# lppllppl920/EndoscopyDepthEstimation-Pytorch

Hardware: AMD Instinct MI355X
Metric: train frame-pairs/sec at 256x320 bs=8 (higher is better)
Workload: dtype f32

## Files before the change

### endoscopydepthestimation-pytorch_amd/csrc/dgrad_newmap_kernels.h

```cpp
#pragma once

#include "dgrad_block_kernels.h"

namespace endo {

template <int NL>
struct NewMapGeom {
    using G = DgradBlockGeom<1, 2, 3, 1, 4>;
    static constexpr int kStage = 12 * G::kCS;
    static constexpr int kW = 9 * 12 * 16;
    static constexpr int kWPre = (kW + kConvThreads - 1) / kConvThreads;
    static constexpr int kConsts = NL * 16 * 4;
    static constexpr size_t kBytes = sizeof(float) * (2 * kStage + NL * kW + kConsts);
    static constexpr int kBlocksPerCu = NL == 1 ? 4 : 3;
    static_assert(kBytes * kBlocksPerCu <= 160 * 1024, "LDS of the resident blocks");
    static_assert(sizeof(double) * 4 * NL * 16 * 2 <= sizeof(float) * kStage, "the final reduction aliases stage 0");
};

template <int NL>
__global__ void __launch_bounds__(kConvThreads, NewMapGeom<NL>::kBlocksPerCu) dgrad_newmap_kernel(const DgradBlockParams p, int tiles_y, int blocks_per_group, int tiles_per_block) {
    using NG = NewMapGeom<NL>;
    using G = typename NG::G;
    constexpr int R = 3;
    extern __shared__ __attribute__((aligned(16))) float smem[];
    float* s_g = smem;
    float* s_w = smem + 2 * NG::kStage;
    float* s_c = s_w + NL * NG::kW;

    const int tid = threadIdx.x;
    const int lane = tid & 63;
    const int wave = __builtin_amdgcn_readfirstlane(tid >> 6);
    const int li = lane & 15;
    const int lk = lane >> 4;
    const int wx = (wave & 1) * 16;
    const int wy = (wave >> 1) * R;

    const int gn = p.group_n > 0 ? p.group_n : p.n;
    const int tps = p.tiles_x * tiles_y;
    const int Q = static_cast<int>(gridDim.x >> 3);
    const bool interleave = (gridDim.x & 7) == 0 && Q > 0 && blocks_per_group % Q == 0;
    int grp, first, t_step, t_last;
    if (interleave) {
        const int lb0 = static_cast<int>(blockIdx.x & 7) * Q;
        grp = lb0 / blocks_per_group;
        const int b0 = lb0 - grp * blocks_per_group;
        first = b0 * tiles_per_block + static_cast<int>(blockIdx.x >> 3);
        t_last = min((b0 + Q) * tiles_per_block, tps * gn);
        t_step = Q;
    } else {
        const int lb = blockIdx.x;
        grp = lb / blocks_per_group;
        first = (lb - grp * blocks_per_group) * tiles_per_block;
        t_last = min(first + tiles_per_block, tps * gn);
        t_step = 1;
    }
    const int ntiles = first < t_last ? (t_last - first + t_step - 1) / t_step : 0;
    if (ntiles <= 0) return;
    const int64_t grp_off = p.group_n > 0 ? grp * p.gs : 0;

    struct Tile { int n, tx, ty, idx; };
    auto place = [&](Tile& t) {
        t.n = t.idx / tps;
        const int rem = t.idx - t.n * tps;
        t.ty = rem / p.tiles_x;
        t.tx = rem - t.ty * p.tiles_x;
    };
    auto advance = [&](Tile& t) { t.idx += t_step; place(t); };
    Tile cur;
    cur.idx = first;
    place(cur);

#pragma unroll
    for (int l = 0; l < NL; ++l) {
        const float* wl = p.wgt[l] + static_cast<int64_t>(p.w_ci_off) * 9;
        const int wcin = p.w_cin[l];
#pragma unroll
        for (int k = 0; k < NG::kWPre; ++k) {
            const int e0 = k * kConvThreads + wave * 64;
            if (e0 < NG::kW) {
                const int e = e0 + lane;
                const int j = e & 15, rest = e >> 4;
                const int tap = rest / 12, cc = rest - tap * 12;
                const bool ok = e < NG::kW && j < p.count;
                const float* src = ok ? wl + cc * 9 * wcin + j * 9 + (8 - tap) : g_pad_consts + 4;
                if (e < NG::kW) __builtin_amdgcn_global_load_lds((gptr_t)src, (lptr_t)(s_w + l * NG::kW + e0), 4, 0, 0);
            }
        }
    }
    const bool co_ok = li < p.count;
    if (tid < NL * 16) {
        const int l = tid >> 4, j = tid & 15;
        const float* sv = p.saved[0];
        const float* ga = p.gamma[0];
        const float* be = p.beta[0];
        if (NL > 1 && l == 1) { sv = p.saved[1]; ga = p.gamma[1]; be = p.beta[1]; }
        if (NL > 2 && l == 2) { sv = p.saved[2]; ga = p.gamma[2]; be = p.beta[2]; }
        f32x4 c4{0.f, 0.f, 0.f, 0.f};
        if (j < p.count) {
            const float mean = sv[grp_off + 2 * j], rstd = sv[grp_off + 2 * j + 1];
            c4 = f32x4{ga[j] * rstd, be[j], mean, rstd};
        }
        *reinterpret_cast<f32x4*>(s_c + tid * 4) = c4;
    }
    const float wfe = p.vg ? (co_ok ? p.vw[li] : 0.f) : 1.f;

    int u_ry[2], u_rx[2];
#pragma unroll
    for (int k = 0; k < 2; ++k) {
        const int u = lane + 64 * k;
        u_ry[k] = u / (G::kCols / 4);
        u_rx[k] = (u - u_ry[k] * (G::kCols / 4)) * 4;
    }
    const bool second_unit = lane + 64 < G::kUnits;
    const unsigned kOob = 0x80000000u;
    unsigned d_vo[2] = {kOob, kOob};
    const float* d_gn = p.g;
    auto dma_tile = [&](const Tile& t) {
        const int x0 = t.tx * G::kTileX, y0 = t.ty * G::kTileY;
#pragma unroll
        for (int k = 0; k < 2; ++k) {
            const int gy = y0 - 1 + u_ry[k], gx = x0 - G::kLeft + u_rx[k];
            const bool ok = gy >= 0 && gy < p.h && gx >= 0 && gx < p.w;
            d_vo[k] = ok ? 4u * static_cast<unsigned>(gy * p.g_w + gx) : kOob;
        }
        d_gn = p.g + grp_off + static_cast<int64_t>(t.n) * p.g_ns;
    };
    auto issue_chunk = [&](int l, int stage) {
        float* dst = s_g + stage * NG::kStage;
        const __amdgpu_buffer_rsrc_t gr = __builtin_amdgcn_make_buffer_rsrc(const_cast<float*>(d_gn), 0, NL * 12 * p.g_cs * 4, 0x00020000);
#pragma unroll
        for (int i = 0; i < 3; ++i) {
            const int c = wave + 4 * i;
            const unsigned so = 4u * static_cast<unsigned>((l * 12 + c) * p.g_cs);
            __builtin_amdgcn_raw_ptr_buffer_load_lds(gr, (lptr_t)(dst + c * G::kCS), 16, d_vo[0], so, 0, 0);
            if (second_unit) __builtin_amdgcn_raw_ptr_buffer_load_lds(gr, (lptr_t)(dst + c * G::kCS + 256), 16, d_vo[1], so, 0, 0);
        }
    };

    f32x4 xc[R], dc[R], total[R];
    const int lane_x = wx + 4 * lk;
    unsigned lo_r[R];
#pragma unroll
    for (int r = 0; r < R; ++r) lo_r[r] = static_cast<unsigned>(li * p.cs + (wy + r) * p.w + lane_x);
    const unsigned lo_ch = static_cast<unsigned>(li * p.cs);
    int64_t cur_off = 0, po_off = 0, cur_voff = 0;
    unsigned cur_rows = 0, po_rows = 0;
    bool cur_full = false, po_full = false;
    auto begin_tile = [&](const Tile& t) {
        const int x0 = t.tx * G::kTileX, y0 = t.ty * G::kTileY;
        cur_full = y0 + G::kTileY <= p.h && x0 + G::kTileX <= p.w;
        cur_off = grp_off + static_cast<int64_t>(t.n) * p.ns + y0 * p.w + x0;
        cur_voff = grp_off + static_cast<int64_t>(t.n) * p.cs + y0 * p.w + x0;
        const float* xb = p.x + cur_off;
        const float* ob = p.vg ? p.vg + cur_voff : p.out + cur_off;
        if (cur_full) {
            cur_rows = co_ok ? 7u : 0u;
#pragma unroll
            for (int r = 0; r < R; ++r) {
                xc[r] = *reinterpret_cast<const f32x4*>(xb + lo_r[r]);
                dc[r] = *reinterpret_cast<const f32x4*>(ob + (p.vg ? lo_r[r] - lo_ch : lo_r[r]));
            }
        } else {
            unsigned rows = 0;
#pragma unroll
            for (int r = 0; r < R; ++r)
                if (y0 + wy + r < p.h) rows |= 1u << r;
            cur_rows = (co_ok && x0 + lane_x + 3 < p.w) ? rows : 0u;
#pragma unroll
            for (int r = 0; r < R; ++r) {
                xc[r] = f32x4{0.f, 0.f, 0.f, 0.f};
                dc[r] = f32x4{0.f, 0.f, 0.f, 0.f};
                if (cur_rows & (1u << r)) {
                    xc[r] = *reinterpret_cast<const f32x4*>(xb + lo_r[r]);
                    dc[r] = *reinterpret_cast<const f32x4*>(ob + (p.vg ? lo_r[r] - lo_ch : lo_r[r]));
                }
            }
        }
    };

    auto store_results = [&]() {
        float* ob = p.out + po_off;
        if (po_full) {
            if (co_ok) {
#pragma unroll
                for (int r = 0; r < R; ++r) *reinterpret_cast<f32x4*>(ob + lo_r[r]) = dc[r];
            }
        } else {
#pragma unroll
            for (int r = 0; r < R; ++r)
                if (po_rows & (1u << r)) *reinterpret_cast<f32x4*>(ob + lo_r[r]) = dc[r];
        }
    };

    constexpr int kFlushTiles = 8;
    float fs1[NL], fs2[NL];
    double ds1[NL], ds2[NL];
    int tiles_since_flush = 0;
#pragma unroll
    for (int l = 0; l < NL; ++l) { fs1[l] = fs2[l] = 0.f; ds1[l] = ds2[l] = 0.0; }
    dma_tile(cur);
    issue_chunk(0, 0);
    Tile nxt = cur;
    advance(nxt);
    int stage = 0;

    for (int t = 0; t < ntiles; ++t) {
#pragma unroll
        for (int l = 0; l < NL; ++l) {
            asm volatile("s_waitcnt vmcnt(0)" ::: "memory");
            __syncthreads();
            if (l == 0) {
                if (t > 0) {
                    store_results();
                }
                begin_tile(cur);
            }
            if (l + 1 < NL) {
                issue_chunk(l + 1, stage ^ 1);
            } else if (t + 1 < ntiles) {
                dma_tile(nxt);
                issue_chunk(0, stage ^ 1);
            }
            f32x4 acc[R];
#pragma unroll
            for (int r = 0; r < R; ++r) acc[r] = f32x4{0.f, 0.f, 0.f, 0.f};
            {
                const float* sg = s_g + stage * NG::kStage;
                const float* wb = s_w + l * NG::kW;
                float av[2][3][R + 2], bw[2][9];
                auto load_quad = [&](int quad, int set) {
                    const float* a_base = sg + (quad * 4 + lk) * G::kCS + wy * G::kCols + wx + li + G::kColOff;
                    const float* b_base = wb + (quad * 4 + lk) * 16 + li;
#pragma unroll
                    for (int r = 0; r < R + 2; ++r)
#pragma unroll
                        for (int dx = 0; dx < 3; ++dx) av[set][dx][r] = a_base[r * G::kCols + dx];
#pragma unroll
                    for (int tap = 0; tap < 9; ++tap) bw[set][tap] = b_base[tap * 12 * 16];
                };
                load_quad(0, 0);
#pragma unroll
                for (int quad = 0; quad < 3; ++quad) {
                    const int set = quad & 1;
                    if (quad + 1 < 3) load_quad(quad + 1, set ^ 1);
                    __builtin_amdgcn_sched_barrier(0);
#pragma unroll
                    for (int dx = 0; dx < 3; ++dx)
#pragma unroll
                        for (int dy = 0; dy < 3; ++dy)
#pragma unroll
                            for (int r = 0; r < R; ++r)
                                acc[r] = __builtin_amdgcn_mfma_f32_16x16x4f32(av[set][dx][r + dy], bw[set][dy * 3 + dx], acc[r], 0, 0, 0);
                    __builtin_amdgcn_sched_barrier(0);
                }
            }
            {
                const f32x4 c4 = *reinterpret_cast<const f32x4*>(s_c + (l * 16 + li) * 4);
                const float scale = c4[0], beta = c4[1], mean = c4[2], rstd = c4[3];
                float s1 = 0.f, s2 = 0.f;
                auto row = [&](int r) {
#pragma unroll
                    for (int e = 0; e < 4; ++e) {
                        const float xcen = xc[r][e] - mean;
                        const float z = fmaf(xcen, scale, beta);
                        const float dz = z > 0.f ? acc[r][e] : 0.f;
                        s1 += dz;
                        s2 = fmaf(dz, xcen, s2);
                        total[r][e] = l == 0 ? scale * dz : fmaf(scale, dz, total[r][e]);
                    }
                };
                if (cur_full) {
#pragma unroll
                    for (int r = 0; r < R; ++r) row(r);
                } else {
#pragma unroll
                    for (int r = 0; r < R; ++r) {
                        if (l == 0) total[r] = f32x4{0.f, 0.f, 0.f, 0.f};
                        if (cur_rows & (1u << r)) row(r);
                    }
                }
                fs1[l] += s1;
                fs2[l] = fmaf(s2, rstd, fs2[l]);
            }
            if (l == NL - 1) {
#pragma unroll
                for (int r = 0; r < R; ++r)
#pragma unroll
                    for (int e = 0; e < 4; ++e) {
                        float old = dc[r][e] * wfe;
                        asm volatile("" : "+v"(old));
                        dc[r][e] = old + total[r][e];
                    }
                po_off = cur_off;
                po_rows = cur_rows;
                po_full = cur_full;
                cur = nxt;
                advance(nxt);
                if (++tiles_since_flush == kFlushTiles) {
                    tiles_since_flush = 0;
#pragma unroll
                    for (int k = 0; k < NL; ++k) {
                        ds1[k] += static_cast<double>(fs1[k]); ds2[k] += static_cast<double>(fs2[k]);
                        fs1[k] = 0.f; fs2[k] = 0.f;
                    }
                }
            }
            stage ^= 1;
            asm volatile("" : "+s"(stage));
        }
    }
    store_results();

    __syncthreads();
    double* red = reinterpret_cast<double*>(smem);
#pragma unroll
    for (int l = 0; l < NL; ++l) {
        double a = ds1[l] + static_cast<double>(fs1[l]), b = ds2[l] + static_cast<double>(fs2[l]);
        a += __shfl_xor(a, 16, 64); a += __shfl_xor(a, 32, 64);
        b += __shfl_xor(b, 16, 64); b += __shfl_xor(b, 32, 64);
        if (lk == 0) {
            red[((wave * NL + l) * 16 + li) * 2] = a;
            red[((wave * NL + l) * 16 + li) * 2 + 1] = b;
        }
    }
    __syncthreads();
    if (tid < 32 * NL) {
        const int l = tid >> 5, j = (tid >> 1) & 15, which = tid & 1;
        if (j < p.count) {
            double t = 0.0;
#pragma unroll
            for (int wv = 0; wv < 4; ++wv) t += red[((wv * NL + l) * 16 + j) * 2 + which];
            double* sc = p.scratch[0];
            if (NL > 1 && l == 1) sc = p.scratch[1];
            if (NL > 2 && l == 2) sc = p.scratch[2];
            atomicAdd(sc + bn_slot_offset(p.slot_stride) + grp_off / 2 + 2 * j + which, t);
        }
    }
}

inline bool dgrad_newmap_ok(const DgradBlockParams& p) {
    return p.count <= 16 && p.acc_from == 0 && 36ll * p.g_cs * 4 < (1ll << 31) && (16ll * p.cs + static_cast<int64_t>(p.h) * p.w) * 4 < (1ll << 32);
}

template <int NL>
inline int launch_dgrad_newmap(DgradBlockParams p, hipStream_t stream) {
    using NG = NewMapGeom<NL>;
    using G = typename NG::G;
    p.tiles_x = (p.w + G::kTileX - 1) / G::kTileX;
    const int tiles_y = (p.h + G::kTileY - 1) / G::kTileY;
    const int groups = p.group_n > 0 ? p.n / p.group_n : 1;
    const int tiles_per_group = p.tiles_x * tiles_y * (p.group_n > 0 ? p.group_n : p.n);
    const int resident = device_cu_count() * NG::kBlocksPerCu / groups;
    const int tiles_per_block = (tiles_per_group + resident - 1) / resident;
    int blocks_per_group = (tiles_per_group + tiles_per_block - 1) / tiles_per_block;
    blocks_per_group = (blocks_per_group + 7) / 8 * 8;
    return launch_dyn(dgrad_newmap_kernel<NL>, dim3(groups * blocks_per_group), kConvThreads, NG::kBytes, stream, p, tiles_y, blocks_per_group, tiles_per_block);
}

}
```

### endoscopydepthestimation-pytorch_amd/csrc/net.hip

```cpp
#include <new>
#include <vector>

#include "dgrad_kernels.h"
#include "dgrad_block_kernels.h"
#include "dgrad_newmap_kernels.h"
#include "td_dgrad_kernels.h"
#include "td_fwd_kernels.h"
#include "wgrad_taps_kernels.h"
#include "wgrad1x1_kernels.h"
#include "wgrad_nsplit_kernels.h"
#include "wgrad_x3_kernels.h"
#include "wgrad_f34_kernels.h"
#include "wgrad_subpix_kernels.h"
#include "wino_fwd_kernels.h"
#include "wino4_fwd_kernels.h"
#include "dgrad_wino_kernels.h"
#include "dgrad_wino3_kernels.h"


namespace endo {

int run_dgrad_wino3_nl4(const DgradBlockParams& p, const float* const* u, hipStream_t stream);
bool dgrad_wino3p_applies(const DgradBlockParams& p);
int run_dgrad_wino3p_nl4(const DgradBlockParams& p, const float* const* u, int blocks, double* fw_parts, int* blocks_used, hipStream_t stream);

constexpr int kGrowth = 12;
constexpr int kLayers = 4;
constexpr int kFirst = 48;
constexpr int kLevels = 5;
constexpr int kNew = kGrowth * kLayers;
constexpr float kBnEps = 1.0e-5f;
constexpr float kBnMomentum = 0.1f;
constexpr int kSideStreamFromLevel = 0;

struct ConvP { int64_t w, b; int cout, cin, ks; int64_t u; int64_t ud; };
struct BnP { int64_t g, b; int c; int64_t run; int64_t saved; };

struct Table {
    ConvP first, final_;
    ConvP down_conv[kLevels][kLayers], td_conv[kLevels], bott_conv[kLayers], tu_conv[kLevels], up_conv[kLevels][kLayers];
    BnP down_bn[kLevels][kLayers], td_bn[kLevels], bott_bn[kLayers], up_bn[kLevels][kLayers];
    std::vector<int64_t> param_offsets;
    std::vector<BnP*> bn_order;
    int64_t param_floats = 0, bn_floats = 0, bn_width_total = 0;
    WinoWeightTable wino;
    WinoWeightTable wino4;
    int64_t wino4_floats = 0;
    int64_t wino_floats = 0;
    WinoDgradTable wino_dgrad;
    int64_t wino_dgrad_floats = 0;
};

inline int down_in(int level) { return kFirst + kNew * level; }
inline int level_channels(int level) { return level < kLevels ? 144 + down_in(level) : 288 + kNew; }

static const Table& table() {
    static Table* t = [] {
        Table* tb = new Table();
        int64_t off = 0;
        auto conv = [&](ConvP& c, int cout, int cin, int ks) {
            c.cout = cout; c.cin = cin; c.ks = ks; c.u = -1; c.ud = -1;
            c.w = off; tb->param_offsets.push_back(off); off += static_cast<int64_t>(cout) * cin * ks * ks;
            c.b = off; tb->param_offsets.push_back(off); off += cout;
        };
        int64_t run = 0, saved = 0;
        auto bn = [&](BnP& b, int c) {
            b.c = c;
            b.g = off; tb->param_offsets.push_back(off); off += c;
            b.b = off; tb->param_offsets.push_back(off); off += c;
            b.run = run; run += 2 * c;
            b.saved = saved; saved += c;
            tb->bn_order.push_back(&b);
        };
        conv(tb->first, kFirst, 3, 3);
        for (int l = 0; l < kLevels; ++l)
            for (int j = 0; j < kLayers; ++j) { bn(tb->down_bn[l][j], down_in(l) + kGrowth * j); conv(tb->down_conv[l][j], kGrowth, down_in(l) + kGrowth * j, 3); }
        for (int l = 0; l < kLevels; ++l) { bn(tb->td_bn[l], down_in(l) + kNew); conv(tb->td_conv[l], down_in(l) + kNew, down_in(l) + kNew, 1); }
        for (int j = 0; j < kLayers; ++j) { bn(tb->bott_bn[j], 288 + kGrowth * j); conv(tb->bott_conv[j], kGrowth, 288 + kGrowth * j, 3); }
        for (int i = 0; i < kLevels; ++i) conv(tb->tu_conv[i], kNew, kNew, 3);
        for (int i = 0; i < kLevels; ++i) {
            const int l = kLevels - 1 - i;
            for (int j = 0; j < kLayers; ++j) { const int cin = 96 + down_in(l) + kGrowth * j; bn(tb->up_bn[i][j], cin); conv(tb->up_conv[i][j], kGrowth, cin, 3); }
        }
        conv(tb->final_, 1, 192, 1);
        tb->param_floats = off;
        tb->bn_floats = run;
        tb->bn_width_total = saved;
        {
            WinoWeightTable& wt = tb->wino;
            wt.layers = 0; wt.start[0] = 0;
            int64_t uoff = 0;
            auto add = [&](ConvP& c) {
                const int l = wt.layers++;
                c.u = uoff;
                wt.cin[l] = c.cin; wt.cout[l] = c.cout; wt.w_off[l] = c.w; wt.u_off[l] = uoff;
                wt.start[l + 1] = wt.start[l] + c.cin * 16;
                uoff += static_cast<int64_t>(c.cin) * kWinoUStride;
            };
            for (int l = 0; l < kLevels; ++l) for (int j = 0; j < kLayers; ++j) add(tb->down_conv[l][j]);
            for (int j = 0; j < kLayers; ++j) add(tb->bott_conv[j]);
            for (int i = 0; i < kLevels; ++i) for (int j = 0; j < kLayers; ++j) add(tb->up_conv[i][j]);
            tb->wino_floats = uoff;
            tb->wino4 = wt;
            int64_t u4 = 0;
            for (int l = 0; l < wt.layers; ++l) { tb->wino4.u_off[l] = u4; u4 += static_cast<int64_t>(wt.cin[l]) * kW4UStride; }
            tb->wino4_floats = u4;
        }
        {
            WinoDgradTable& wd = tb->wino_dgrad;
            wd.layers = 0; wd.start[0] = 0;
            int64_t uoff = 0;
            auto add = [&](ConvP& c, int base) {
                const int l = wd.layers++;
                c.ud = uoff;
                wd.cin[l] = c.cin; wd.groups[l] = base / 16; wd.w_off[l] = c.w; wd.u_off[l] = uoff;
                wd.start[l + 1] = wd.start[l] + 16 * wd.groups[l] * 12;
                uoff += static_cast<int64_t>(wd.groups[l]) * kWinoDgradSlice;
            };
            for (int l = 0; l < kLevels; ++l) for (int j = 0; j < kLayers; ++j) add(tb->down_conv[l][j], down_in(l));
            for (int j = 0; j < kLayers; ++j) add(tb->bott_conv[j], 288);
            for (int i = 0; i < kLevels; ++i) for (int j = 0; j < kLayers; ++j) add(tb->up_conv[i][j], 96 + down_in(kLevels - 1 - i));
            tb->wino_dgrad_floats = uoff;
        }
        return tb;
    }();
    return *t;
}

}

using namespace endo;

struct endo_net {
    int n, h, w;
    int groups;
    int64_t gs;
    struct Level { int h, w, t; int64_t plane; int64_t act, grad; int64_t sums; int64_t pq; } lv[kLevels + 1];
    int64_t pre_off;
    int64_t saved_off;
    int64_t idx_off[kLevels];
    int64_t sums_off;
    int64_t sums_bytes;
    int64_t tape_floats;
    int64_t partial_off;
    int64_t wino_off;
    int64_t wino4_off;
    int64_t pq_off;
    int64_t pq_floats;
    int64_t scratch_off;
    int64_t scratch_bytes;
    int64_t slot_stride;
    int64_t wg_scratch_off;
    int64_t tuw_scratch_off;
    int64_t wd_off;
    int64_t gplane_off;
    int64_t bias_parts_off;
    int64_t fw_parts_off;
    int64_t bias_parts_floats;
    int64_t gradws_floats;
    hipStream_t wstream;
    hipEvent_t ev_fork, ev_join;
    int opt[ENDO_OPT_COUNT];
};

namespace endo {


constexpr int kBiasPartChannels = 2048;
constexpr int kBiasPartLaunches = 64;
constexpr int kFwPartBlocks = 512;
struct BiasReduceTable {
    int n;
    struct Entry { const float* parts; float* bias; int count; int nparts; } e[kBiasPartLaunches];
};
struct BiasParts {
    BiasReduceTable table;
    int64_t used;
};

struct BnFin4 {
    const double* scratch[4];
    const float* saved[4];
    const float* gamma[4];
    float* ggamma[4];
    float* gbeta[4];
};

__global__ void __launch_bounds__(256) prep_dy_kernel(float* __restrict__ dbuf, const float* __restrict__ x, int64_t ns, int plane,
                                                      const float* __restrict__ pq_p, const float* __restrict__ pq_q,
                                                      float* bias_grad, int group_n, int64_t gs, const BnFin4 fin, int nl,
                                                      double count, int training, int64_t slot_stride,
                                                      const float* __restrict__ vg, const float* __restrict__ vw, float* __restrict__ parts) {
    __shared__ double scratch[4];
    const int c = blockIdx.y;
    const int grp = blockIdx.z / group_n, n = blockIdx.z - grp * group_n;
    float pc = pq_p[grp * gs + c], qc = pq_q[grp * gs + c];
    if (nl > 0) {
        const int64_t go = grp * gs;
        double dp = 0.0, dq = 0.0;
#pragma unroll
        for (int j = 0; j < 4; ++j) {
            if (j >= nl) break;
            const double s1 = bn_slot_sum(fin.scratch[j] + go / 2 + 2 * c, slot_stride);
            const double s2 = bn_slot_sum(fin.scratch[j] + go / 2 + 2 * c + 1, slot_stride);
            if (blockIdx.x == 0 && n == 0 && threadIdx.x == 0) {
                atomicAdd(fin.ggamma[j] + c, static_cast<float>(s2));
                atomicAdd(fin.gbeta[j] + c, static_cast<float>(s1));
            }
            if (training) {
                const double mean = fin.saved[j][go + 2 * c], rstd = fin.saved[j][go + 2 * c + 1];
                const double scale = fin.gamma[j][c] * rstd;
                const double k = scale * rstd * s2 / count;
                dp += static_cast<double>(static_cast<float>(-k));
                dq += static_cast<double>(static_cast<float>(-scale * s1 / count + k * mean));
            }
        }
        pc += static_cast<float>(dp);
        qc += static_cast<float>(dq);
    }
    const int64_t base = grp * gs + n * ns + static_cast<int64_t>(c) * plane;
    const float* vg_n = vg ? vg + grp * gs + static_cast<int64_t>(n) * plane : nullptr;
    const float wf = vg ? vw[c] : 0.f;
    float part = 0.f;
    if ((plane & 3) == 0 && !vg_n) {
        const int stride = gridDim.x * blockDim.x * 4;
        int i = (blockIdx.x * blockDim.x + threadIdx.x) * 4;
        for (; i + stride < plane; i += 2 * stride) {
            f32x4 g0 = *reinterpret_cast<const f32x4*>(dbuf + base + i);
            f32x4 g1 = *reinterpret_cast<const f32x4*>(dbuf + base + i + stride);
            const f32x4 x0 = *reinterpret_cast<const f32x4*>(x + base + i);
            const f32x4 x1 = *reinterpret_cast<const f32x4*>(x + base + i + stride);
#pragma unroll
            for (int e = 0; e < 4; ++e) { g0[e] += fmaf(pc, x0[e], qc); part += g0[e]; }
#pragma unroll
            for (int e = 0; e < 4; ++e) { g1[e] += fmaf(pc, x1[e], qc); part += g1[e]; }
            *reinterpret_cast<f32x4*>(dbuf + base + i) = g0;
            *reinterpret_cast<f32x4*>(dbuf + base + i + stride) = g1;
        }
        for (; i < plane; i += stride) {
            f32x4 g = *reinterpret_cast<const f32x4*>(dbuf + base + i);
            const f32x4 xv = *reinterpret_cast<const f32x4*>(x + base + i);
#pragma unroll
            for (int e = 0; e < 4; ++e) { g[e] += fmaf(pc, xv[e], qc); part += g[e]; }
            *reinterpret_cast<f32x4*>(dbuf + base + i) = g;
        }
    } else if ((plane & 3) == 0) {
        for (int i = (blockIdx.x * blockDim.x + threadIdx.x) * 4; i < plane; i += gridDim.x * blockDim.x * 4) {
            f32x4 g;
            if (vg_n) {
                const f32x4 gv = *reinterpret_cast<const f32x4*>(vg_n + i);
                g = f32x4{gv[0] * wf, gv[1] * wf, gv[2] * wf, gv[3] * wf};
            } else {
                g = *reinterpret_cast<const f32x4*>(dbuf + base + i);
            }
            const f32x4 xv = *reinterpret_cast<const f32x4*>(x + base + i);
#pragma unroll
            for (int e = 0; e < 4; ++e) { g[e] += fmaf(pc, xv[e], qc); part += g[e]; }
            *reinterpret_cast<f32x4*>(dbuf + base + i) = g;
        }
    } else {
        for (int i = blockIdx.x * blockDim.x + threadIdx.x; i < plane; i += gridDim.x * blockDim.x) {
            const float g = (vg_n ? vg_n[i] * wf : dbuf[base + i]) + fmaf(pc, x[base + i], qc);
            dbuf[base + i] = g;
            part += g;
        }
    }
    const int lane = threadIdx.x & 63, wave = threadIdx.x >> 6;
    double v = wave_sum(static_cast<double>(part));
    if (lane == 0) scratch[wave] = v;
    __syncthreads();
    if (threadIdx.x == 0 && bias_grad) {
        const float t = static_cast<float>(scratch[0] + scratch[1] + scratch[2] + scratch[3]);
        if (parts) parts[(static_cast<int64_t>(c) * gridDim.z + blockIdx.z) * gridDim.x + blockIdx.x] = t;
        else atomicAdd(bias_grad + c, t);
    }
}

__global__ void __launch_bounds__(256) bias_reduce_kernel(const BiasReduceTable tb) {
    const BiasReduceTable::Entry& e = tb.e[blockIdx.x];
    const int lane = threadIdx.x & 63, wave = threadIdx.x >> 6;
    for (int c = blockIdx.y * 4 + wave; c < e.count; c += gridDim.y * 4) {
        const float* src = e.parts + static_cast<int64_t>(c) * e.nparts;
        double t = 0.0;
        for (int i = lane; i < e.nparts; i += 64) t += static_cast<double>(src[i]);
        t = wave_sum(t);
        if (lane == 0) e.bias[c] += static_cast<float>(t);
    }
}

__global__ void bn_bwd_finalize_kernel(const double* __restrict__ scratch, const float* __restrict__ saved,
                                       const float* __restrict__ gamma, float* __restrict__ ggamma, float* __restrict__ gbeta,
                                       float* __restrict__ pq_p, float* __restrict__ pq_q, int c_count, double count, int training,
                                       int64_t gs, int64_t slot_stride) {
    scratch += blockIdx.y * (gs / 2); saved += blockIdx.y * gs; pq_p += blockIdx.y * gs; pq_q += blockIdx.y * gs;
    for (int c = blockIdx.x * blockDim.x + threadIdx.x; c < c_count; c += gridDim.x * blockDim.x) {
        const double s1 = bn_slot_sum(scratch + 2 * c, slot_stride), s2 = bn_slot_sum(scratch + 2 * c + 1, slot_stride);
        atomicAdd(ggamma + c, static_cast<float>(s2));
        atomicAdd(gbeta + c, static_cast<float>(s1));
        if (training) {
            const double mean = saved[2 * c], rstd = saved[2 * c + 1];
            const double scale = gamma[c] * rstd;
            const double k = scale * rstd * s2 / count;
            pq_p[c] += static_cast<float>(-k);
            pq_q[c] += static_cast<float>(-scale * s1 / count + k * mean);
        }
    }
}

__global__ void bn_bwd_finalize4_kernel(const BnFin4 a, int nl, float* __restrict__ pq_p, float* __restrict__ pq_q, int c_count, double count,
                                        int training, int64_t gs, int64_t slot_stride) {
    const int64_t go = blockIdx.y * gs;
    pq_p += go; pq_q += go;
    for (int c = blockIdx.x * blockDim.x + threadIdx.x; c < c_count; c += gridDim.x * blockDim.x) {
        double dp = 0.0, dq = 0.0;
#pragma unroll
        for (int j = 0; j < 4; ++j) {
            if (j >= nl) break;
            const double s1 = bn_slot_sum(a.scratch[j] + go / 2 + 2 * c, slot_stride);
            const double s2 = bn_slot_sum(a.scratch[j] + go / 2 + 2 * c + 1, slot_stride);
            atomicAdd(a.ggamma[j] + c, static_cast<float>(s2));
            atomicAdd(a.gbeta[j] + c, static_cast<float>(s1));
            if (training) {
                const double mean = a.saved[j][go + 2 * c], rstd = a.saved[j][go + 2 * c + 1];
                const double scale = a.gamma[j][c] * rstd;
                const double k = scale * rstd * s2 / count;
                dp += static_cast<double>(static_cast<float>(-k));
                dq += static_cast<double>(static_cast<float>(-scale * s1 / count + k * mean));
            }
        }
        if (training) {
            pq_p[c] += static_cast<float>(dp);
            pq_q[c] += static_cast<float>(dq);
        }
    }
}

__global__ void tu_phase_weights_kernel(const float* __restrict__ w, int cout, int cin, float* __restrict__ out) {
    constexpr int kPhW = 2 * 12 * 16 + 16;
    const int total = 2 * cin * 2 * 12 * 16;
    for (int i = blockIdx.x * blockDim.x + threadIdx.x; i < total; i += gridDim.x * blockDim.x) {
        const int lane16 = i & 15;
        const int slot = (i >> 4) % 12;
        const int t = (i / (16 * 12)) & 1;
        const int ci = (i / (16 * 12 * 2)) % cin;
        const int a = i / (16 * 12 * 2 * cin);
        int ctap, tile;
        if (slot < 3) { ctap = 0; tile = slot; } else if (slot < 9) { ctap = 1; tile = slot - 3; } else { ctap = 2; tile = slot - 9 + 3; }
        const int b = tile / 3, co = (tile % 3) * 16 + lane16;
        float v = 0.f;
        if (co < cout) {
            const float* src = w + (static_cast<int64_t>(co) * cin + ci) * 9;
            const int ky0 = a == 0 ? (t == 0 ? 0 : 1) : (t == 0 ? 0 : 2), ky1 = a == 0 ? (t == 0 ? 0 : 2) : (t == 0 ? 1 : 2);
            int kx0, kx1;
            if (b == 0) { kx0 = ctap == 0 ? 0 : 1; kx1 = ctap == 0 ? 0 : 2; }
            else { kx0 = ctap == 1 ? 0 : 2; kx1 = ctap == 1 ? 1 : 2; }
            for (int ky = ky0; ky <= ky1; ++ky)
                for (int kx = kx0; kx <= kx1; ++kx) v += src[ky * 3 + kx];
        }
        out[(static_cast<int64_t>(a) * cin + ci) * kPhW + (t * 12 + slot) * 16 + lane16] = v;
    }
}

__global__ void tu_subpix_dgrad_weights_kernel(const float* __restrict__ w, int cout, int cin, float* __restrict__ out) {
    const int pitch = 4 * cin + 16;
    const int total = 4 * cout * 4 * cin;
    for (int i = blockIdx.x * blockDim.x + threadIdx.x; i < total; i += gridDim.x * blockDim.x) {
        const int ci = i % cin;
        const int tap = (i / cin) & 3;
        const int co = (i / (4 * cin)) % cout;
        const int ph = i / (4 * cin * cout);
        const int alpha = ph >> 1, beta = ph & 1, tyi = tap >> 1, txi = tap & 1;
        const int ky0 = alpha == 0 ? (tyi == 0 ? 1 : 0) : (tyi == 0 ? 2 : 0), ky1 = alpha == 0 ? (tyi == 0 ? 2 : 0) : (tyi == 0 ? 2 : 1);
        const int kx0 = beta == 0 ? (txi == 0 ? 1 : 0) : (txi == 0 ? 2 : 0), kx1 = beta == 0 ? (txi == 0 ? 2 : 0) : (txi == 0 ? 2 : 1);
        const float* src = w + (static_cast<int64_t>(co) * cin + ci) * 9;
        float v = 0.f;
        for (int ky = ky0; ky <= ky1; ++ky)
            for (int kx = kx0; kx <= kx1; ++kx) v += src[ky * 3 + kx];
        out[static_cast<int64_t>(ph * cout + co) * pitch + tap * cin + ci] = v;
    }
}

__global__ void __launch_bounds__(256) finalize_partial_kernel(const float* __restrict__ partial, int64_t split_stride, int ksplit,
                                                               int64_t pns, int plane, const float* __restrict__ bias,
                                                               float* __restrict__ out, int64_t out_ns, double* out_sums,
                                                               int group_n, int64_t gs) {
    __shared__ double scratch[2 * 4];
    const int c = blockIdx.y;
    const int grp = blockIdx.z / group_n, n = blockIdx.z - grp * group_n;
    partial += grp * gs; out += grp * gs;
    if (out_sums) out_sums += grp * (gs / 2);
    const float b = bias[c];
    float part[2] = {0.f, 0.f};
    for (int i = blockIdx.x * blockDim.x + threadIdx.x; i < plane; i += gridDim.x * blockDim.x) {
        float v = b;
        for (int s = 0; s < ksplit; ++s) v += partial[s * split_stride + n * pns + static_cast<int64_t>(c) * plane + i];
        out[n * out_ns + static_cast<int64_t>(c) * plane + i] = v;
        part[0] += v;
        part[1] += v * v;
    }
    if (out_sums) block_sum_atomic<2>(part, out_sums + 2 * c, scratch);
}

__global__ void __launch_bounds__(256) final_fwd_kernel(const float* __restrict__ u, int64_t ns, int plane, int cin,
                                                        const float* __restrict__ wgt, const float* __restrict__ bias,
                                                        float* __restrict__ pre, float* __restrict__ out, int group_n, int64_t gs, int c_first) {
    __shared__ float s_w[192];
    for (int c = threadIdx.x; c < cin; c += blockDim.x) s_w[c] = wgt[c];
    __syncthreads();
    const int grp = blockIdx.y / group_n, n = blockIdx.y - grp * group_n;
    u += grp * gs;
    if (pre) pre += grp * gs;
    out += static_cast<int64_t>(grp) * group_n * plane;
    const bool vec = (plane & 3) == 0;
    if (vec) {
        for (int i = (blockIdx.x * blockDim.x + threadIdx.x) * 4; i < plane; i += gridDim.x * blockDim.x * 4) {
            f32x4 acc = {0.f, 0.f, 0.f, 0.f};
            if (c_first > 0) acc = *reinterpret_cast<const f32x4*>(pre + static_cast<int64_t>(n) * plane + i);
            const float* src = u + n * ns + i;
            for (int c = c_first; c < cin; ++c) {
                const f32x4 v = *reinterpret_cast<const f32x4*>(src + static_cast<int64_t>(c) * plane);
                const float wc = s_w[c];
                acc[0] = fmaf(v[0], wc, acc[0]); acc[1] = fmaf(v[1], wc, acc[1]);
                acc[2] = fmaf(v[2], wc, acc[2]); acc[3] = fmaf(v[3], wc, acc[3]);
            }
            const float b = bias[0];
            f32x4 o;
            for (int e = 0; e < 4; ++e) { acc[e] += b; o[e] = fabsf(acc[e]); }
            if (pre) *reinterpret_cast<f32x4*>(pre + static_cast<int64_t>(n) * plane + i) = acc;
            *reinterpret_cast<f32x4*>(out + static_cast<int64_t>(n) * plane + i) = o;
        }
    } else {
        for (int i = blockIdx.x * blockDim.x + threadIdx.x; i < plane; i += gridDim.x * blockDim.x) {
            float acc = c_first > 0 ? pre[static_cast<int64_t>(n) * plane + i] : 0.f;
            for (int c = c_first; c < cin; ++c) acc = fmaf(u[n * ns + static_cast<int64_t>(c) * plane + i], s_w[c], acc);
            acc += bias[0];
            if (pre) pre[static_cast<int64_t>(n) * plane + i] = acc;
            out[static_cast<int64_t>(n) * plane + i] = fabsf(acc);
        }
    }
}

__device__ __forceinline__ float sign_of(float v) { return v > 0.f ? 1.f : (v < 0.f ? -1.f : 0.f); }

__global__ void __launch_bounds__(256) final_g_kernel(const float* __restrict__ gout, const float* __restrict__ pre, float* __restrict__ g,
                                                      int plane, int group_n, int64_t gs) {
    const int grp = blockIdx.y / group_n, n = blockIdx.y - grp * group_n;
    gout += static_cast<int64_t>(blockIdx.y) * plane; pre += grp * gs + static_cast<int64_t>(n) * plane; g += grp * gs + static_cast<int64_t>(n) * plane;
    for (int i = blockIdx.x * blockDim.x + threadIdx.x; i < plane; i += gridDim.x * blockDim.x) g[i] = gout[i] * sign_of(pre[i]);
}

__global__ void __launch_bounds__(256) final_bwd_data_kernel(const float* __restrict__ gout, const float* __restrict__ pre,
                                                             const float* __restrict__ wgt, float* __restrict__ dbuf,
                                                             int64_t ns, int plane, int cin, int group_n, int64_t gs, int c_first) {
    __shared__ float s_w[192];
    for (int c = threadIdx.x; c < cin; c += blockDim.x) s_w[c] = wgt[c];
    __syncthreads();
    const int grp = blockIdx.y / group_n, n = blockIdx.y - grp * group_n;
    gout += static_cast<int64_t>(grp) * group_n * plane; pre += grp * gs; dbuf += grp * gs;
    for (int i = blockIdx.x * blockDim.x + threadIdx.x; i < plane; i += gridDim.x * blockDim.x) {
        const float g = gout[static_cast<int64_t>(n) * plane + i] * sign_of(pre[static_cast<int64_t>(n) * plane + i]);
        for (int c = c_first; c < cin; ++c) dbuf[n * ns + static_cast<int64_t>(c) * plane + i] = g * s_w[c];
    }
}

__global__ void __launch_bounds__(256) final_bwd_weight_kernel(const float* __restrict__ gout, const float* __restrict__ pre,
                                                               const float* __restrict__ u, int64_t ns, int plane, int cin,
                                                               int group_n, int64_t gs, float* __restrict__ gw, float* __restrict__ gb, int c_first) {
    __shared__ double scratch[4];
    const int c = c_first + blockIdx.x;
    const int grp = blockIdx.z / group_n, n = blockIdx.z - grp * group_n;
    const float* gp = gout + static_cast<int64_t>(blockIdx.z) * plane;
    const float* pp = pre + grp * gs + static_cast<int64_t>(n) * plane;
    const float* up = u + grp * gs + n * ns + static_cast<int64_t>(c < cin ? c : 0) * plane;
    float part = 0.f, part2 = 0.f;
    if ((plane & 3) == 0) {
        const int stride = gridDim.y * blockDim.x * 4;
        for (int i = (blockIdx.y * blockDim.x + threadIdx.x) * 4; i < plane; i += stride) {
            const f32x4 gv = *reinterpret_cast<const f32x4*>(gp + i);
            const f32x4 pv = *reinterpret_cast<const f32x4*>(pp + i);
            f32x4 uv = {1.f, 1.f, 1.f, 1.f};
            if (c < cin) uv = *reinterpret_cast<const f32x4*>(up + i);
            part += gv[0] * sign_of(pv[0]) * uv[0] + gv[1] * sign_of(pv[1]) * uv[1];
            part2 += gv[2] * sign_of(pv[2]) * uv[2] + gv[3] * sign_of(pv[3]) * uv[3];
        }
    } else {
        for (int i = blockIdx.y * blockDim.x + threadIdx.x; i < plane; i += gridDim.y * blockDim.x)
            part += gp[i] * sign_of(pp[i]) * (c < cin ? up[i] : 1.f);
    }
    const int lane = threadIdx.x & 63, wave = threadIdx.x >> 6;
    double v = wave_sum(static_cast<double>(part + part2));
    if (lane == 0) scratch[wave] = v;
    __syncthreads();
    if (threadIdx.x == 0) {
        const float t = static_cast<float>(scratch[0] + scratch[1] + scratch[2] + scratch[3]);
        if (c < cin) atomicAdd(gw + c, t); else atomicAdd(gb, t);
    }
}

__global__ void __launch_bounds__(64) final_w_reduce_kernel(const double* __restrict__ parts, int nblocks, int count, float* __restrict__ gw) {
    const int c = blockIdx.x;
    double t = 0.0;
    for (int b = threadIdx.x; b < nblocks; b += 64) t += parts[static_cast<int64_t>(b) * count + c];
    t = wave_sum(t);
    if (threadIdx.x == 0) atomicAdd(gw + c, static_cast<float>(t));
}

constexpr int kBlocks = 2 * kLevels + 1, kDense = kBlocks * kLayers;

enum class DenseFwd { Wino4, Wino2_32x16, Wino2_32x8, SplitK, Direct32x8, Direct16x8, DirectAuto };
struct FwdPlan {
    struct Dense {
        DenseFwd form;
        int stages;
        int ksplit;
        bool chunk_weights;
    } dense[kDense];
    bool bf16;
    bool wino4_weights;
    bool fuse_final;
    bool td_persistent[kLevels];
    bool tu_subpix[kLevels];
};

enum class NewMap { Bf16, Persistent, Vec16, Dword };
enum class BasePass { Block8, Block8Bf16, Wino3, Wino3Persistent, Wino8 };
enum class DenseWgrad { F34, X3, NSplit, Taps, Direct };
enum class TdDgrad { Persistent, Runs128, Dma, Staged };
enum class TuWgrad { Subpix, Taps, Direct };
enum class TuDgrad { Subpix32x8, Subpix16x8, Subpix16x4, Plain };
enum class FirstWgrad { F34Prep, F34, Taps, Direct };
struct BwdPlan {
    struct Block {
        bool fused;
        NewMap newmap[kLayers];
        BasePass base;
        bool wino3_layout;
    } block[kBlocks];
    DenseWgrad wgrad[kDense];
    bool td_wgrad_dma[kLevels];
    TdDgrad td_dgrad[kLevels];
    TuWgrad tu_wgrad[kLevels];
    TuDgrad tu_dgrad[kLevels];
    int overlap;
    bool bf16_wgrad, bf16_dgrad;
    int f34_blocks;
    bool dgrad_weights;
    bool use_virt;
    bool virt_base;
    bool virt_base_w;
    int materialise;
    int c_first;
    FirstWgrad first;
};

struct Ctx {
    const endo_net* net;
    const float* params;
    float* bn_running;
    float* tape;
    float* grads;
    float* gradws;
    int training;
    hipStream_t stream;
    BiasParts* bias_parts = nullptr;
    const float* x = nullptr;
    const FwdPlan* fwd = nullptr;
    const BwdPlan* bwd = nullptr;

    int nt() const { return net->n * net->groups; }
    int fork_wgrad(Ctx& side, int level) const {
        side = *this;
        if (!net->wstream || !bwd->overlap || level < kSideStreamFromLevel) return 0;
        ENDO_CHECK(hipEventRecord(net->ev_fork, stream));
        ENDO_CHECK(hipStreamWaitEvent(net->wstream, net->ev_fork, 0));
        side.stream = net->wstream;
        return 0;
    }
    float* act(int level) const { return tape + net->lv[level].act; }
    float* gbuf(int level) const { return gradws + net->lv[level].grad; }
    double* sums(int level) const { return reinterpret_cast<double*>(reinterpret_cast<char*>(tape) + net->sums_off) + net->lv[level].sums; }
    double* out_sums(int level, int channel) const { return training ? sums(level) + 2 * channel : nullptr; }
    float* saved(const BnP& b) const { return tape + net->saved_off + 2 * b.saved; }
    double* scratch(const BnP& b) const { return reinterpret_cast<double*>(reinterpret_cast<char*>(gradws) + net->scratch_off) + 2 * b.saved; }
    float* pq_p(int level) const { return gradws + net->pq_off + 2 * net->lv[level].pq; }
    float* pq_q(int level) const { return pq_p(level) + net->lv[level].t; }
    uint8_t* idx(int level) const { return reinterpret_cast<uint8_t*>(tape) + net->idx_off[level]; }
};

static void fill_bn_in(const Ctx& c, ConvParams& p, const BnP& b, int level, int ic0) {
    const auto& lv = c.net->lv[level];
    p.in_sums = c.sums(level) + 2 * ic0;
    p.gamma = c.params + b.g;
    p.beta = c.params + b.b;
    p.running_mean = c.bn_running + b.run;
    p.running_var = c.bn_running + b.run + b.c;
    p.saved = c.tape ? c.saved(b) : nullptr;
    p.count = static_cast<double>(c.net->n) * lv.h * lv.w;
    p.eps = kBnEps;
    p.momentum = kBnMomentum;
    p.training = c.training;
}

static void fill_in(const Ctx& c, ConvParams& p, const float* base, int level, int ic0, int cin) {
    const auto& lv = c.net->lv[level];
    p.in = base + ic0 * lv.plane;
    p.in_ns = lv.t * lv.plane;
    p.in_cs = static_cast<int>(lv.plane);
    p.in_w = lv.w;
    p.cin = cin;
}

static void fill_out(const Ctx& c, ConvParams& p, float* base, int level, int oc0, int cout) {
    const auto& lv = c.net->lv[level];
    p.out = base + oc0 * lv.plane;
    p.out_ns = lv.t * lv.plane;
    p.out_cs = static_cast<int>(lv.plane);
    p.out_w = lv.w;
    p.cout = cout;
}

static void fill_grid(const Ctx& c, ConvParams& p, int level) {
    const auto& lv = c.net->lv[level];
    p.n = c.nt(); p.h = lv.h; p.w = lv.w;
    p.group_n = c.net->n; p.gs = c.net->gs; p.in_gs = c.net->gs; p.out_gs = c.net->gs;
}

static double conv_flops(const endo_net* net, int level, int cin, int cout, int ks) {
    return 2.0 * net->n * net->groups * net->lv[level].plane * cin * cout * ks * ks;
}

static void default_options(int (&opt)[ENDO_OPT_COUNT]) {
    opt[ENDO_OPT_WINO_FWD] = 5;
    opt[ENDO_OPT_WINO_DGRAD] = 3;
    opt[ENDO_OPT_DGRAD_VEC] = 2;
    opt[ENDO_OPT_WINO_MIN_TILES] = 1024;
    opt[ENDO_OPT_MFMA_BF16] = 0;
    opt[ENDO_OPT_WGRAD_OVERLAP] = 1;
    opt[ENDO_OPT_MFMA_X3] = 0;
    opt[ENDO_OPT_WGRAD_F34] = 1;
    opt[ENDO_OPT_FINAL_VIRTUAL] = 1;
    opt[ENDO_OPT_TD_PERSIST] = 3;
}
static int bf16_mask(const int* opt) { const int v = opt[ENDO_OPT_MFMA_BF16]; return v == 1 ? 7 : (v >> 1); }

struct DenseBlock { int level, ic0, c0; const BnP* bn; const ConvP* cv; bool base_overwrite; };
static DenseBlock dense_block(int b) {
    const Table& tb = table();
    if (b < kLevels) return {b, 48, down_in(b), tb.down_bn[b], tb.down_conv[b], false};
    if (b == kLevels) return {kLevels, 0, 288, tb.bott_bn, tb.bott_conv, true};
    const int i = b - kLevels - 1, l = kLevels - 1 - i;
    return {l, 0, 96 + down_in(l), tb.up_bn[i], tb.up_conv[i], l > 0};
}
static long tile_count(const Ctx& c, int level, int tx, int ty) {
    const auto& lv = c.net->lv[level];
    return static_cast<long>((lv.w + tx - 1) / tx) * ((lv.h + ty - 1) / ty) * c.nt();
}

static ConvParams dense_fwd_params(const Ctx& c, const DenseBlock& k, int j, DenseFwd form) {
    const ConvP& cv = k.cv[j];
    const int oc0 = k.ic0 + k.c0 + kGrowth * j;
    ConvParams p{};
    fill_grid(c, p, k.level);
    fill_in(c, p, c.act(k.level), k.level, k.ic0, cv.cin);
    fill_bn_in(c, p, k.bn[j], k.level, k.ic0);
    p.wgt = c.params + cv.w; p.bias = c.params + cv.b; p.w_cout = cv.cout; p.w_cin = cv.cin;
    fill_out(c, p, c.act(k.level), k.level, oc0, cv.cout);
    p.out_sums = c.out_sums(k.level, oc0);
    if (form == DenseFwd::Wino4) p.wgt = c.tape + c.net->wino4_off + cv.u / kWinoUStride * kW4UStride;
    if (form == DenseFwd::Wino2_32x16 || form == DenseFwd::Wino2_32x8) p.wgt = c.tape + c.net->wino_off + cv.u;
    return p;
}

static ConvParams td_fwd_params(const Ctx& c, int level) {
    const BnP& b = table().td_bn[level];
    const ConvP& cv = table().td_conv[level];
    const int next = level + 1;
    const int oc0 = next < kLevels ? 48 : 0;
    ConvParams p{};
    fill_grid(c, p, level);
    fill_in(c, p, c.act(level), level, 48, cv.cin);
    fill_bn_in(c, p, b, level, 48);
    p.wgt = c.params + cv.w; p.bias = c.params + cv.b; p.w_cout = cv.cout; p.w_cin = cv.cin;
    fill_out(c, p, c.act(next), next, oc0, cv.cout);
    p.out_idx = c.idx(level);
    p.idx_ns = static_cast<int64_t>(cv.cout) * c.net->lv[next].plane;
    p.out_sums = c.out_sums(next, oc0);
    return p;
}

static FwdPlan plan_fwd(const Ctx& c) {
    const int* opt = c.net->opt;
    const int mode = opt[ENDO_OPT_WINO_FWD];
    const long min_tiles = opt[ENDO_OPT_WINO_MIN_TILES];
    FwdPlan pl{};
    pl.bf16 = (bf16_mask(opt) & 2) != 0;
    pl.wino4_weights = !pl.bf16 && mode == 5;
    for (int b = 0; b < kBlocks; ++b) {
        const DenseBlock k = dense_block(b);
        const long t64x16 = tile_count(c, k.level, 64, 16), t32x16 = tile_count(c, k.level, 32, 16), t32x8 = tile_count(c, k.level, 32, 8);
        const long t16x16 = tile_count(c, k.level, 16, 16), t16x8 = tile_count(c, k.level, 16, 8);
        const bool big = t32x16 >= min_tiles, small = t32x8 >= (min_tiles * 3) / 4;
        const bool wino4_tiles = mode == 5 && !pl.bf16 && 2 * t64x16 >= min_tiles;
        const bool wino2_tiles = mode != 0 && !pl.bf16 && (big || small);
        for (int j = 0; j < kLayers; ++j) {
            FwdPlan::Dense& d = pl.dense[b * kLayers + j];
            const int nchunks = (k.cv[j].cin + 15) / 16;
            d.chunk_weights = !pl.bf16 && !wino4_tiles && !wino2_tiles;
            d.stages = mode == 4 ? 4 : (mode == 3 ? 3 : 2);
            if (wino4_tiles && wino4_fwd_ok(dense_fwd_params(c, k, j, DenseFwd::Wino4))) {
                d.form = DenseFwd::Wino4;
            } else if (wino2_tiles && wino_fwd_ok(dense_fwd_params(c, k, j, DenseFwd::Wino2_32x16))) {
                d.form = big ? DenseFwd::Wino2_32x16 : DenseFwd::Wino2_32x8;
            } else if (t32x16 < 512 && t16x16 < 384 && t16x8 < 512 && nchunks >= 4) {
                int want = static_cast<int>(((t16x8 < 256 ? 512 : 768) + t16x8 - 1) / t16x8);
                if (want > nchunks) want = nchunks;
                const int per = (nchunks + want - 1) / want;
                d.form = DenseFwd::SplitK;
                d.ksplit = (nchunks + per - 1) / per;
            } else {
                d.form = (t32x16 < 1024 && t32x8 >= 1024) ? DenseFwd::Direct32x8
                       : (t32x16 < 1024 && t16x8 >= 768) ? DenseFwd::Direct16x8 : DenseFwd::DirectAuto;
            }
        }
    }
    pl.fuse_final = opt[ENDO_OPT_FINAL_VIRTUAL] && pl.dense[kDense - 1].form == DenseFwd::Wino4;
    for (int l = 0; l < kLevels; ++l) {
        pl.td_persistent[l] = (opt[ENDO_OPT_TD_PERSIST] & 2) && !pl.bf16 && c.training && td_fwd_ok(td_fwd_params(c, l));
        const ConvP& tu = table().tu_conv[kLevels - 1 - l];
        pl.tu_subpix[l] = c.net->lv[l + 1].w % 4 == 0 && tu.cout == kNew && tu.cin % 4 == 0;
    }
    return pl;
}

static int dense_fwd(const Ctx& c, int b, int j) {
    const DenseBlock k = dense_block(b);
    const FwdPlan::Dense& d = c.fwd->dense[b * kLayers + j];
    const ConvP& cv = k.cv[j];
    const auto& lv = c.net->lv[k.level];
    const int oc0 = k.ic0 + k.c0 + kGrowth * j;
    ConvParams p = dense_fwd_params(c, k, j, d.form);
    ProfScope prof(kProfConv3x3Dense, c.stream, conv_flops(c.net, k.level, cv.cin, cv.cout, 3),
                   4.0 * c.nt() * lv.plane * (cv.cin + cv.cout));
    const float* chunk_weights = d.chunk_weights ? c.tape + c.net->wino_off + cv.u : nullptr;
    const bool bf16 = c.fwd->bf16;
    switch (d.form) {
        case DenseFwd::Wino4:
            if (c.fwd->fuse_final && b == kBlocks - 1 && j == kLayers - 1) { p.fin_w = c.params + table().final_.w + k.ic0; p.fin_out = c.tape + c.net->pre_off; }
            return launch_wino4_fwd(p, c.stream);
        case DenseFwd::Wino2_32x16:
            return d.stages == 4 ? launch_wino_fwd<2, 4, 2, 4>(p, c.stream) : d.stages == 3 ? launch_wino_fwd<2, 4, 2, 3>(p, c.stream) : launch_wino_fwd<2, 4, 2, 2>(p, c.stream);
        case DenseFwd::Wino2_32x8:
            return d.stages == 4 ? launch_wino_fwd<1, 4, 3, 4>(p, c.stream) : d.stages == 3 ? launch_wino_fwd<1, 4, 3, 3>(p, c.stream) : launch_wino_fwd<1, 4, 3, 2>(p, c.stream);
        case DenseFwd::SplitK: {
            float* partial = c.tape + c.net->partial_off;
            p.ksplit = d.ksplit;
            p.split_stride = static_cast<int64_t>(c.net->n) * cv.cout * lv.plane;
            p.out = partial; p.out_ns = static_cast<int64_t>(cv.cout) * lv.plane;
            p.bias = nullptr; p.out_sums = nullptr;
            p.wgt_chunks = chunk_weights;
            int rc = bf16 ? launch_conv_dma<3, 16, 1, IN_BNRELU, EPI_FWD, 1, 2, 2, 1, 1>(p, c.stream)
                          : launch_conv_dma<3, 16, 1, IN_BNRELU, EPI_FWD, 1, 2, 2, 1>(p, c.stream);
            if (rc) return rc;
            int bx = static_cast<int>((lv.plane + 255) / 256);
            bx = bx > 8 ? 8 : bx;
            finalize_partial_kernel<<<dim3(bx, cv.cout, c.nt()), 256, 0, c.stream>>>(
                partial, p.split_stride, d.ksplit, p.out_ns, static_cast<int>(lv.plane), c.params + cv.b, c.act(k.level) + oc0 * lv.plane,
                lv.t * lv.plane, c.out_sums(k.level, oc0), c.net->n, c.net->gs);
            ENDO_LAUNCH_CHECK();
            return 0;
        }
        case DenseFwd::Direct32x8:
            return bf16 ? launch_conv_dma<3, 4, 1, IN_BNRELU, EPI_FWD, 2, 4, 2, 1, 1>(p, c.stream) : launch_conv_dma<3, 4, 1, IN_BNRELU, EPI_FWD, 2, 4, 2, 1>(p, c.stream);
        case DenseFwd::Direct16x8:
            return bf16 ? launch_conv_dma<3, 8, 1, IN_BNRELU, EPI_FWD, 1, 2, 2, 1, 1>(p, c.stream) : launch_conv_dma<3, 8, 1, IN_BNRELU, EPI_FWD, 1, 2, 2, 1>(p, c.stream);
        case DenseFwd::DirectAuto:
            if (bf16) return launch_conv_dma_auto<3, 4, 1, IN_BNRELU, EPI_FWD, 8, 2, 1, 1>(p, c.stream);
            p.wgt_chunks = chunk_weights;
            return launch_conv_dma_auto<3, 4, 1, IN_BNRELU, EPI_FWD, 8, 2, 1>(p, c.stream);
    }
    return ENDO_E_BADARG;
}

static int td_fwd(const Ctx& c, int level) {
    const ConvP& cv = table().td_conv[level];
    const ConvParams p = td_fwd_params(c, level);
    ProfScope prof(kProfConv1x1Pool, c.stream, conv_flops(c.net, level, cv.cin, cv.cout, 1),
                   4.0 * c.nt() * c.net->lv[level].plane * (cv.cin + cv.cout / 4.0));
    if (c.fwd->td_persistent[level]) return launch_td_fwd(p, device_cu_count(), c.stream);
    if (c.fwd->bf16) return launch_conv_dma_auto<1, 8, 3, IN_BNRELU, EPI_FWD_POOL, 4, 2, 1, 1>(p, c.stream);
    return launch_conv_dma_auto<1, 8, 3, IN_BNRELU, EPI_FWD_POOL, 4>(p, c.stream);
}

static int tu_fwd(const Ctx& c, int level, int src_level, int src_c0, const ConvP& cv) {
    ProfScope prof(kProfConv3x3Up, c.stream, conv_flops(c.net, level, cv.cin, cv.cout, 3),
                   4.0 * c.nt() * c.net->lv[level].plane * (cv.cin / 4.0 + cv.cout));
    if (c.fwd->tu_subpix[level]) {
        float* w3 = c.tape + c.net->partial_off;
        tu_phase_weights_kernel<<<(2 * cv.cin * 384 + 255) / 256, 256, 0, c.stream>>>(c.params + cv.w, cv.cout, cv.cin, w3);
        ENDO_LAUNCH_CHECK();
        ConvParams p{};
        fill_grid(c, p, src_level);
        fill_in(c, p, c.act(src_level), src_level, src_c0, cv.cin);
        p.wgt = w3; p.w_cout = 2 * cv.cout; p.w_cin = cv.cin;
        p.bias = c.params + cv.b;
        fill_out(c, p, c.act(level), level, 0, cv.cout);
        p.out_sums = c.out_sums(level, 0);
        return launch_conv_dma_vec<3, 4, 6, IN_PLAIN, EPI_FWD, 2, 4, 2, 1, 4, 0, 0, 2>(p, c.stream);
    }
    ConvParams p{};
    fill_grid(c, p, level);
    fill_in(c, p, c.act(src_level), src_level, src_c0, cv.cin);
    p.wgt = c.params + cv.w; p.bias = c.params + cv.b; p.w_cout = cv.cout; p.w_cin = cv.cin;
    fill_out(c, p, c.act(level), level, 0, cv.cout);
    p.out_sums = c.out_sums(level, 0);
    return launch_conv_dma_auto<3, 4, 3, IN_UPSAMPLE, EPI_FWD>(p, c.stream);
}

struct FinalVirt { const float* vg; const float* vw; float* gw; };

static int prep_dy(const Ctx& c, int level, int c0, int count, float* bias_grad, const BnFin4* fin = nullptr, int nl = 0, const FinalVirt* fv = nullptr) {
    const auto& lv = c.net->lv[level];
    BnFin4 none{};
    int bx = static_cast<int>((lv.plane + 4095) / 4096);
    bx = bx < 1 ? 1 : (bx > 32 ? 32 : bx);
    float* parts = nullptr;
    if (bias_grad && c.bias_parts) {
        BiasParts& bp = *c.bias_parts;
        const int64_t need = static_cast<int64_t>(count) * c.nt() * bx;
        if (bp.table.n >= kBiasPartLaunches || bp.used + need > c.net->bias_parts_floats) return ENDO_E_UNSUPPORTED;
        parts = c.gradws + c.net->bias_parts_off + bp.used;
        bp.table.e[bp.table.n++] = {parts, bias_grad, count, c.nt() * bx};
        bp.used += need;
    }
    ProfScope prof(kProfSmall, c.stream, 0.0, 12.0 * c.nt() * lv.plane * count);
    prep_dy_kernel<<<dim3(bx, count, c.nt()), 256, 0, c.stream>>>(c.gbuf(level) + c0 * lv.plane, c.act(level) + c0 * lv.plane,
                                                                     lv.t * lv.plane, static_cast<int>(lv.plane), c.pq_p(level) + c0,
                                                                     c.pq_q(level) + c0, bias_grad, c.net->n, c.net->gs, fin ? *fin : none, fin ? nl : 0,
                                                                     static_cast<double>(c.net->n) * lv.h * lv.w, c.training, c.net->slot_stride,
                                                                     fv ? fv->vg : nullptr, fv ? fv->vw + c0 : nullptr, parts);
    ENDO_LAUNCH_CHECK();
    return 0;
}

static int bn_finalize(const Ctx& c, const BnP& b, int level, int ic0, int first = 0, int count = -1) {
    const auto& lv = c.net->lv[level];
    if (count < 0) count = b.c - first;
    if (count <= 0) return 0;
    ProfScope prof(kProfSmall, c.stream, 0.0, 0.0);
    bn_bwd_finalize_kernel<<<dim3((count + 127) / 128, c.net->groups), 128, 0, c.stream>>>(c.scratch(b) + 2 * first, c.saved(b) + 2 * first, c.params + b.g + first,
                                                                       c.grads + b.g + first, c.grads + b.b + first,
                                                                       c.pq_p(level) + ic0 + first, c.pq_q(level) + ic0 + first, count,
                                                                       static_cast<double>(c.net->n) * lv.h * lv.w, c.training, c.net->gs, c.net->slot_stride);
    ENDO_LAUNCH_CHECK();
    return 0;
}

static void fill_wgrad_grid(const Ctx& c, WgradParams& p, int level) {
    const auto& lv = c.net->lv[level];
    p.n = c.nt(); p.h = lv.h; p.w = lv.w;
    p.group_n = c.net->n; p.gs = c.net->gs; p.in_gs = c.net->gs;
    p.tiles_x = (lv.w + kWgTileX - 1) / kWgTileX;
    p.tiles_y = (lv.h + kWgTileY - 1) / kWgTileY;
}

static WgradParams dense_wgrad_params(const Ctx& c, const DenseBlock& k, int j) {
    const auto& lv = c.net->lv[k.level];
    const BnP& b = k.bn[j];
    const ConvP& cv = k.cv[j];
    const int oc0 = k.ic0 + k.c0 + kGrowth * j;
    WgradParams p{};
    fill_wgrad_grid(c, p, k.level);
    p.in = c.act(k.level) + k.ic0 * lv.plane; p.in_ns = lv.t * lv.plane; p.in_cs = static_cast<int>(lv.plane); p.in_w = lv.w; p.cin = cv.cin;
    p.saved = c.saved(b); p.gamma = c.params + b.g; p.beta = c.params + b.b;
    p.dy = c.gbuf(k.level) + oc0 * lv.plane; p.dy_ns = lv.t * lv.plane; p.dy_cs = static_cast<int>(lv.plane); p.dy_w = lv.w; p.cout = cv.cout;
    p.dw = c.grads + cv.w;
    return p;
}

static void fill_dgrad_block(const Ctx& c, DgradBlockParams& p, int level) {
    const auto& lv = c.net->lv[level];
    p.n = c.nt(); p.h = lv.h; p.w = lv.w;
    p.group_n = c.net->n; p.gs = c.net->gs; p.slot_stride = c.net->slot_stride;
    p.g_ns = lv.t * lv.plane; p.g_cs = static_cast<int>(lv.plane); p.g_w = lv.w;
    p.ns = lv.t * lv.plane; p.cs = static_cast<int>(lv.plane);
}

static DgradBlockParams newmap_params(const Ctx& c, const DenseBlock& k, int j, BnFin4* a = nullptr) {
    const auto& lv = c.net->lv[k.level];
    const int nl = kLayers - j;
    const int t0 = k.c0 + kGrowth * (j - 1);
    DgradBlockParams p{};
    fill_dgrad_block(c, p, k.level);
    p.g = c.gbuf(k.level) + (k.ic0 + k.c0 + kGrowth * j) * lv.plane;
    p.x = c.act(k.level) + (k.ic0 + t0) * lv.plane;
    p.out = c.gbuf(k.level) + (k.ic0 + t0) * lv.plane;
    p.count = kGrowth;
    p.acc_from = 0;
    p.w_ci_off = t0;
    for (int l = 0; l < nl; ++l) {
        const BnP& b = k.bn[j + l];
        p.wgt[l] = c.params + k.cv[j + l].w; p.w_cin[l] = k.cv[j + l].cin;
        p.saved[l] = c.saved(b) + 2 * t0; p.gamma[l] = c.params + b.g + t0; p.beta[l] = c.params + b.b + t0;
        p.scratch[l] = c.scratch(b) + 2 * t0;
        if (a) { a->scratch[l] = p.scratch[l]; a->saved[l] = p.saved[l]; a->gamma[l] = p.gamma[l]; a->ggamma[l] = c.grads + b.g + t0; a->gbeta[l] = c.grads + b.b + t0; }
    }
    return p;
}

static DgradBlockParams base_pass_params(const Ctx& c, const DenseBlock& k) {
    const auto& lv = c.net->lv[k.level];
    DgradBlockParams p{};
    fill_dgrad_block(c, p, k.level);
    p.g = c.gbuf(k.level) + (k.ic0 + k.c0) * lv.plane;
    p.x = c.act(k.level) + k.ic0 * lv.plane;
    p.out = c.gbuf(k.level) + k.ic0 * lv.plane;
    p.count = k.c0;
    p.acc_from = k.base_overwrite ? k.c0 : 0;
    p.w_ci_off = 0;
    for (int j = 0; j < kLayers; ++j) {
        p.wgt[j] = c.params + k.cv[j].w; p.w_cin[j] = k.cv[j].cin;
        p.saved[j] = c.saved(k.bn[j]); p.gamma[j] = c.params + k.bn[j].g; p.beta[j] = c.params + k.bn[j].b;
        p.scratch[j] = c.scratch(k.bn[j]);
    }
    return p;
}

static WgradParams td_wgrad_params(const Ctx& c, int level) {
    const BnP& b = table().td_bn[level];
    const ConvP& cv = table().td_conv[level];
    const int next = level + 1, oc0 = next < kLevels ? 48 : 0;
    const auto& lv = c.net->lv[level];
    const auto& nx = c.net->lv[next];
    WgradParams p{};
    fill_wgrad_grid(c, p, level);
    p.in = c.act(level) + 48 * lv.plane; p.in_ns = lv.t * lv.plane; p.in_cs = static_cast<int>(lv.plane); p.in_w = lv.w; p.cin = cv.cin;
    p.saved = c.saved(b); p.gamma = c.params + b.g; p.beta = c.params + b.b;
    p.dy = c.gbuf(next) + oc0 * nx.plane; p.dy_ns = nx.t * nx.plane; p.dy_cs = static_cast<int>(nx.plane); p.dy_w = nx.w; p.cout = cv.cout;
    p.dy_idx = c.idx(level); p.idx_ns = static_cast<int64_t>(cv.cout) * nx.plane;
    p.dw = c.grads + cv.w;
    return p;
}

static ConvParams td_dgrad_params(const Ctx& c, int level) {
    const BnP& b = table().td_bn[level];
    const ConvP& cv = table().td_conv[level];
    const int next = level + 1, oc0 = next < kLevels ? 48 : 0;
    const auto& lv = c.net->lv[level];
    ConvParams p{};
    fill_grid(c, p, level);
    fill_in(c, p, c.gbuf(next), next, oc0, cv.cout);
    p.in_idx = c.idx(level); p.idx_ns = static_cast<int64_t>(cv.cout) * c.net->lv[next].plane;
    p.wgt = c.params + cv.w; p.w_cout = cv.cout; p.w_cin = cv.cin;
    fill_out(c, p, c.gbuf(level), level, 48, cv.cin);
    p.x = c.act(level) + 48 * lv.plane; p.x_ns = lv.t * lv.plane; p.x_cs = static_cast<int>(lv.plane);
    p.bn_saved = c.saved(b); p.bn_gamma = c.params + b.g; p.bn_beta = c.params + b.b;
    p.bn_scratch = c.scratch(b); p.bn_slot_stride = c.net->slot_stride;
    p.acc_from = 0;
    return p;
}

static WgradParams tu_wgrad_params(const Ctx& c, int level, bool subpix) {
    const ConvP& cv = table().tu_conv[kLevels - 1 - level];
    const int src_level = level + 1, src_c0 = src_level == kLevels ? 288 : 96 + down_in(src_level);
    const auto& lv = c.net->lv[level];
    const auto& sv = c.net->lv[src_level];
    WgradParams p{};
    fill_wgrad_grid(c, p, level);
    p.in = c.act(src_level) + src_c0 * sv.plane; p.in_ns = sv.t * sv.plane; p.in_cs = static_cast<int>(sv.plane); p.in_w = sv.w; p.cin = cv.cin;
    p.dy = c.gbuf(level); p.dy_ns = lv.t * lv.plane; p.dy_cs = static_cast<int>(lv.plane); p.dy_w = lv.w; p.cout = cv.cout;
    p.dw = c.grads + cv.w;
    if (subpix) { p.h = sv.h; p.w = sv.w; }
    return p;
}

static WgradParams first_wgrad_params(const Ctx& c) {
    const auto& lv = c.net->lv[0];
    WgradParams p{};
    fill_wgrad_grid(c, p, 0);
    p.in = c.x; p.in_ns = 3 * lv.plane; p.in_cs = static_cast<int>(lv.plane); p.in_w = lv.w; p.cin = 3;
    p.in_gs = c.net->n * p.in_ns;
    p.dy = c.gbuf(0) + 48 * lv.plane; p.dy_ns = lv.t * lv.plane; p.dy_cs = static_cast<int>(lv.plane); p.dy_w = lv.w; p.cout = kFirst;
    p.dw = c.grads + table().first.w;
    return p;
}

static BwdPlan plan_bwd(const Ctx& c) {
    const int* opt = c.net->opt;
    const int wino_dgrad = opt[ENDO_OPT_WINO_DGRAD];
    const long min_tiles = opt[ENDO_OPT_WINO_MIN_TILES];
    BwdPlan pl{};
    pl.overlap = opt[ENDO_OPT_WGRAD_OVERLAP];
    pl.bf16_wgrad = (bf16_mask(opt) & 1) != 0;
    pl.bf16_dgrad = (bf16_mask(opt) & 4) != 0;
    const bool x3 = !pl.bf16_wgrad && (opt[ENDO_OPT_MFMA_X3] & 1);
    const bool f34 = opt[ENDO_OPT_WGRAD_F34] && !pl.bf16_wgrad && !x3;
    const long f34_min_tiles = min_tiles / 4;
    pl.f34_blocks = opt[ENDO_OPT_WGRAD_F34] == 2 ? 256 : kF34Blocks;
    pl.dgrad_weights = wino_dgrad != 0 && !pl.bf16_dgrad;
    for (int b = 0; b < kBlocks; ++b) {
        const DenseBlock k = dense_block(b);
        const auto& lv = c.net->lv[k.level];
        BwdPlan::Block& bl = pl.block[b];
        const DgradBlockParams base = base_pass_params(c, k);
        bl.fused = dgrad_block_ok(base);
        const long wtiles = static_cast<long>(lv.w / 32) * (lv.h / 8) * c.nt();
        if (pl.bf16_dgrad) bl.base = BasePass::Block8Bf16;
        else if (wino_dgrad != 0 && dgrad_wino_ok(base) && wtiles >= min_tiles)
            bl.base = !((wino_dgrad == 1 || wino_dgrad == 3) && dgrad_wino3_ok(base)) ? BasePass::Wino8
                    : (wino_dgrad == 3 && dgrad_wino3p_applies(base)) ? BasePass::Wino3Persistent : BasePass::Wino3;
        else bl.base = BasePass::Block8;
        bl.wino3_layout = bl.base == BasePass::Wino3 || bl.base == BasePass::Wino3Persistent;
        for (int j = 1; j < kLayers; ++j) {
            const DgradBlockParams p = newmap_params(c, k, j);
            const bool vec = dgrad_block_vec_ok(p);
            bl.newmap[j] = (pl.bf16_dgrad && vec) ? NewMap::Bf16 : (vec && opt[ENDO_OPT_DGRAD_VEC] >= 2 && dgrad_newmap_ok(p)) ? NewMap::Persistent
                         : (vec && opt[ENDO_OPT_DGRAD_VEC] != 0) ? NewMap::Vec16 : NewMap::Dword;
        }
        for (int j = 0; j < kLayers; ++j) {
            const WgradParams p = dense_wgrad_params(c, k, j);
            pl.wgrad[b * kLayers + j] = (f34 && wgrad_f34_ok(p, f34_min_tiles)) ? DenseWgrad::F34 : wgrad_nsplit_ok(p) ? (x3 ? DenseWgrad::X3 : DenseWgrad::NSplit)
                                      : wgrad_taps_ok(p) ? DenseWgrad::Taps : DenseWgrad::Direct;
        }
    }
    for (int l = 0; l < kLevels; ++l) {
        const auto& sv = c.net->lv[l + 1];
        pl.td_wgrad_dma[l] = wgrad1x1_dma_ok(td_wgrad_params(c, l));
        const ConvParams td = td_dgrad_params(c, l);
        const bool persist = (opt[ENDO_OPT_TD_PERSIST] & 1) && !pl.bf16_dgrad;
        pl.td_dgrad[l] = (persist && td_dgrad_ok(td)) ? TdDgrad::Persistent : (persist && sv.w % 4 != 0 && td_dgrad_small_ok(td)) ? TdDgrad::Runs128
                       : sv.w % 4 == 0 ? TdDgrad::Dma : TdDgrad::Staged;
        const ConvP& tu = table().tu_conv[kLevels - 1 - l];
        pl.tu_wgrad[l] = tu_wgrad_subpix_ok(tu_wgrad_params(c, l, true)) ? TuWgrad::Subpix : wgrad_taps_ok(tu_wgrad_params(c, l, false), true) ? TuWgrad::Taps : TuWgrad::Direct;
        pl.tu_dgrad[l] = !(sv.w % 4 == 0 && tu.cin == kNew && tu.cout == kNew) ? TuDgrad::Plain : tile_count(c, l + 1, 32, 8) >= 1024 ? TuDgrad::Subpix32x8
                       : tile_count(c, l + 1, 16, 8) >= 512 ? TuDgrad::Subpix16x8 : TuDgrad::Subpix16x4;
    }
    const BwdPlan::Block& last = pl.block[kBlocks - 1];
    const int last_base = dense_block(kBlocks - 1).c0;
    pl.use_virt = opt[ENDO_OPT_FINAL_VIRTUAL] && last.fused;
    pl.virt_base = pl.use_virt && last.wino3_layout;
    pl.virt_base_w = pl.use_virt && last.base == BasePass::Wino3Persistent;
    pl.materialise = !pl.use_virt ? 192 : (pl.virt_base ? 0 : last_base);
    pl.c_first = pl.virt_base_w ? last_base : 0;
    const WgradParams first = first_wgrad_params(c);
    pl.first = (f34 && wgrad_f34_raw_ok(first, f34_min_tiles)) ? (opt[ENDO_OPT_FINAL_VIRTUAL] ? FirstWgrad::F34Prep : FirstWgrad::F34)
             : wgrad_taps_ok(first) ? FirstWgrad::Taps : FirstWgrad::Direct;
    return pl;
}

static int dense_wgrad(const Ctx& c, int b, int j, F34ReduceBatch* batch = nullptr, int slice = 0) {
    const DenseBlock k = dense_block(b);
    const ConvP& cv = k.cv[j];
    const auto& lv = c.net->lv[k.level];
    const WgradParams p = dense_wgrad_params(c, k, j);
    float* scratch = c.gradws + c.net->wg_scratch_off;
    ProfScope prof(kProfWgradDense, c.stream, conv_flops(c.net, k.level, cv.cin, cv.cout, 3), 4.0 * c.nt() * lv.plane * (cv.cin + cv.cout));
    switch (c.bwd->wgrad[b * kLayers + j]) {
        case DenseWgrad::F34: return launch_wgrad_f34(p, scratch + (batch ? slice : 0) * kF34ScratchFloats, c.stream, c.bwd->f34_blocks, batch);
        case DenseWgrad::X3: return launch_wgrad_x3(p, scratch, c.stream);
        case DenseWgrad::NSplit: return launch_wgrad_nsplit(p, scratch, c.stream, c.bwd->bf16_wgrad ? 1 : 0);
        case DenseWgrad::Taps: return c.bwd->bf16_wgrad ? launch_wgrad_taps<12, IN_BNRELU, 1>(p, c.stream) : launch_wgrad_taps<12, IN_BNRELU>(p, c.stream);
        case DenseWgrad::Direct: return launch_wgrad<3, 1, IN_BNRELU, DY_PLAIN>(p, c.stream);
    }
    return ENDO_E_BADARG;
}

static int dense_bwd(const Ctx& c, int b, int j, int acc_from) {
    const DenseBlock k = dense_block(b);
    const BnP& bn = k.bn[j];
    const ConvP& cv = k.cv[j];
    const int level = k.level, ic0 = k.ic0, oc0 = k.ic0 + k.c0 + kGrowth * j;
    const auto& lv = c.net->lv[level];
    int rc = prep_dy(c, level, oc0, cv.cout, c.grads + cv.b);
    if (rc) return rc;
    {
        Ctx cw;
        rc = c.fork_wgrad(cw, level);
        if (rc) return rc;
        rc = dense_wgrad(cw, b, j);
        if (rc) return rc;
    }
    {
        ConvParams p{};
        fill_grid(c, p, level);
        fill_in(c, p, c.gbuf(level), level, oc0, cv.cout);
        p.wgt = c.params + cv.w; p.w_cout = cv.cout; p.w_cin = cv.cin;
        fill_out(c, p, c.gbuf(level), level, ic0, cv.cin);
        p.x = c.act(level) + ic0 * lv.plane; p.x_ns = lv.t * lv.plane; p.x_cs = static_cast<int>(lv.plane);
        p.bn_saved = c.saved(bn); p.bn_gamma = c.params + bn.g; p.bn_beta = c.params + bn.b;
        p.bn_scratch = c.scratch(bn); p.bn_slot_stride = c.net->slot_stride;
        p.acc_from = acc_from - ic0;
        ProfScope prof(kProfDgradDense, c.stream, conv_flops(c.net, level, cv.cin, cv.cout, 3), 4.0 * c.nt() * lv.plane * (3.0 * cv.cin + cv.cout));
        rc = launch_dgrad_dense_auto(p, c.stream);
        if (rc) return rc;
    }
    return bn_finalize(c, bn, level, ic0);
}

template <int NL>
static int launch_newmap(NewMap form, const DgradBlockParams& p, hipStream_t stream) {
    switch (form) {
        case NewMap::Bf16: return launch_dgrad_block<NL, 2, 3, 1, 0, 1, 4, 1>(p, stream);
        case NewMap::Persistent: return launch_dgrad_newmap<NL>(p, stream);
        case NewMap::Vec16: return launch_dgrad_block<NL, 2, 3, 1, 0, 1, 4>(p, stream);
        case NewMap::Dword: return launch_dgrad_block<NL, 2, 3>(p, stream);
    }
    return ENDO_E_BADARG;
}

static int dense_block_bwd(const Ctx& c, int b, const FinalVirt* fv = nullptr) {
    const DenseBlock k = dense_block(b);
    const BwdPlan::Block& bl = c.bwd->block[b];
    const int level = k.level, ic0 = k.ic0, c0 = k.c0, new0 = ic0 + c0;
    const auto& lv = c.net->lv[level];
    if (!bl.fused) {
        for (int j = kLayers - 1; j >= 0; --j) {
            const int acc_from = (j == kLayers - 1 && k.base_overwrite) ? new0 : 0;
            int rc = dense_bwd(c, b, j, acc_from < ic0 ? ic0 : acc_from);
            if (rc) return rc;
        }
        return 0;
    }
    BnFin4 pending{};
    int pending_nl = 0;
    F34ReduceBatch red{};
    for (int j = kLayers - 1; j >= 0; --j) {
        int rc = prep_dy(c, level, new0 + kGrowth * j, kGrowth, c.grads + k.cv[j].b, &pending, pending_nl, (fv && j == kLayers - 1) ? fv : nullptr);
        if (rc) return rc;
        const bool defer = c.bwd->overlap == 2;
        if (!defer || j == 0) {
            Ctx cw;
            rc = c.fork_wgrad(cw, level);
            if (rc) return rc;
            for (int jj = defer ? kLayers - 1 : j; jj >= j; --jj) {
                rc = dense_wgrad(cw, b, jj, &red, jj);
                if (rc) return rc;
            }
            if (j == 0 && red.count > 0) {
                ProfScope prof(kProfSmall, cw.stream, 0.0, 0.0);
                rc = launch_wgrad_f34_reduce_batch(red, cw.stream);
                if (rc) return rc;
            }
        }
        if (j > 0) {
            const int nl = kLayers - j;
            BnFin4 a{};
            DgradBlockParams p = newmap_params(c, k, j, &a);
            if (fv) { p.vg = fv->vg; p.vw = fv->vw + ic0 + p.w_ci_off; }
            ProfScope prof(kProfDgradDense, c.stream, 2.0 * c.nt() * lv.plane * kGrowth * kGrowth * 9 * nl,
                           4.0 * c.nt() * lv.plane * (3.0 * kGrowth + kGrowth * nl));
            rc = nl == 1 ? launch_newmap<1>(bl.newmap[j], p, c.stream) : nl == 2 ? launch_newmap<2>(bl.newmap[j], p, c.stream) : launch_newmap<3>(bl.newmap[j], p, c.stream);
            if (rc) return rc;
            pending = a;
            pending_nl = nl;
        }
    }
    {
        DgradBlockParams p = base_pass_params(c, k);
        const bool virt = fv && c.bwd->virt_base;
        if (virt) { p.vg = fv->vg; p.vw = fv->vw + ic0; }
        ProfScope prof(kProfDgradDense, c.stream, 2.0 * c.nt() * lv.plane * c0 * kGrowth * 9 * kLayers,
                       4.0 * c.nt() * lv.plane * (3.0 * c0 + kGrowth * kLayers));
        const float* ub = c.gradws + c.net->wd_off;
        const float* const u[4] = {ub + k.cv[0].ud, ub + k.cv[1].ud, ub + k.cv[2].ud, ub + k.cv[3].ud};
        int rc = 0;
        switch (bl.base) {
            case BasePass::Block8Bf16: rc = launch_dgrad_block8<4, 1>(p, c.stream); break;
            case BasePass::Block8: rc = launch_dgrad_block8<4>(p, c.stream); break;
            case BasePass::Wino8: rc = launch_dgrad_wino8<4>(p, u, c.stream); break;
            case BasePass::Wino3: rc = run_dgrad_wino3_nl4(p, u, c.stream); break;
            case BasePass::Wino3Persistent: {
                double* fwp = (virt && c.bwd->virt_base_w) ? reinterpret_cast<double*>(c.gradws + c.net->fw_parts_off) : nullptr;
                int used = 0;
                rc = run_dgrad_wino3p_nl4(p, u, std::min(device_cu_count(), kFwPartBlocks), fwp, &used, c.stream);
                if (rc == 0 && fwp) {
                    final_w_reduce_kernel<<<c0, 64, 0, c.stream>>>(fwp, used, c0, fv->gw + ic0);
                    ENDO_LAUNCH_CHECK();
                }
                break;
            }
        }
        if (rc) return rc;
    }
    {
        BnFin4 a;
        for (int j = 0; j < kLayers; ++j) {
            a.scratch[j] = c.scratch(k.bn[j]); a.saved[j] = c.saved(k.bn[j]); a.gamma[j] = c.params + k.bn[j].g;
            a.ggamma[j] = c.grads + k.bn[j].g; a.gbeta[j] = c.grads + k.bn[j].b;
        }
        ProfScope prof(kProfSmall, c.stream, 0.0, 0.0);
        bn_bwd_finalize4_kernel<<<dim3((c0 + 127) / 128, c.net->groups), 128, 0, c.stream>>>(a, kLayers, c.pq_p(level) + ic0, c.pq_q(level) + ic0, c0,
                                                                         static_cast<double>(c.net->n) * lv.h * lv.w, c.training, c.net->gs,
                                                                         c.net->slot_stride);
        ENDO_LAUNCH_CHECK();
    }
    return 0;
}

static int td_bwd(const Ctx& c, int level) {
    const BnP& b = table().td_bn[level];
    const ConvP& cv = table().td_conv[level];
    const int next = level + 1;
    const auto& lv = c.net->lv[level];
    int rc = prep_dy(c, next, next < kLevels ? 48 : 0, cv.cout, c.grads + cv.b);
    if (rc) return rc;
    {
        const WgradParams p = td_wgrad_params(c, level);
        Ctx cw;
        rc = c.fork_wgrad(cw, level);
        if (rc) return rc;
        ProfScope prof(kProfWgradOther, cw.stream, conv_flops(c.net, level, cv.cin, cv.cout, 1), 4.0 * c.nt() * lv.plane * cv.cin);
        rc = !c.bwd->td_wgrad_dma[level] ? launch_wgrad1x1(p, cw.stream) : c.bwd->bf16_wgrad ? launch_wgrad1x1_dma<1>(p, cw.stream) : launch_wgrad1x1_dma<0>(p, cw.stream);
        if (rc) return rc;
    }
    {
        const ConvParams p = td_dgrad_params(c, level);
        ProfScope prof(kProfDgradOther, c.stream, conv_flops(c.net, level, cv.cin, cv.cout, 1), 4.0 * c.nt() * lv.plane * 3.0 * cv.cin);
        switch (c.bwd->td_dgrad[level]) {
            case TdDgrad::Persistent: rc = launch_td_dgrad(p, device_cu_count(), c.stream); break;
            case TdDgrad::Runs128: rc = launch_td_dgrad_small(p, c.stream); break;
            case TdDgrad::Dma: rc = c.bwd->bf16_dgrad ? launch_conv_dma_auto<1, 16, 2, IN_UNPOOL, EPI_DGRAD_BN, 4, 2, 1, 1>(p, c.stream)
                                                      : launch_conv_dma_auto<1, 16, 2, IN_UNPOOL, EPI_DGRAD_BN, 4>(p, c.stream); break;
            case TdDgrad::Staged: rc = launch_conv_auto<1, 16, 3, IN_UNPOOL, EPI_DGRAD_BN, 4>(p, c.stream); break;
        }
        if (rc) return rc;
    }
    return bn_finalize(c, b, level, 48);
}

static int tu_bwd(const Ctx& c, int level, int src_level, int src_c0, const ConvP& cv) {
    const auto& lv = c.net->lv[level];
    int rc = prep_dy(c, level, 0, cv.cout, c.grads + cv.b);
    if (rc) return rc;
    {
        const TuWgrad form = c.bwd->tu_wgrad[level];
        const WgradParams p = tu_wgrad_params(c, level, form == TuWgrad::Subpix);
        Ctx cw;
        rc = c.fork_wgrad(cw, level);
        if (rc) return rc;
        ProfScope prof(kProfWgradOther, cw.stream, conv_flops(c.net, level, cv.cin, cv.cout, 3), 4.0 * c.nt() * lv.plane * (cv.cin / 4.0 + cv.cout));
        rc = form == TuWgrad::Subpix ? launch_tu_wgrad_subpix(p, c.gradws + c.net->wg_scratch_off, cw.stream)
           : form == TuWgrad::Taps ? launch_wgrad_taps<12, IN_UPSAMPLE>(p, cw.stream) : launch_wgrad<3, 1, IN_UPSAMPLE, DY_PLAIN>(p, cw.stream);
        if (rc) return rc;
    }
    ProfScope prof(kProfDgradOther, c.stream, conv_flops(c.net, level, cv.cin, cv.cout, 3), 4.0 * c.nt() * lv.plane * (cv.cout + cv.cin / 4.0));
    const TuDgrad form = c.bwd->tu_dgrad[level];
    if (form == TuDgrad::Plain) {
        ConvParams p{};
        fill_grid(c, p, level);
        fill_in(c, p, c.gbuf(level), level, 0, cv.cout);
        p.wgt = c.params + cv.w; p.w_cout = cv.cout; p.w_cin = cv.cin;
        fill_out(c, p, c.gbuf(src_level), src_level, src_c0, cv.cin);
        return launch_conv_dma_auto<3, 4, 3, IN_PLAIN, EPI_DGRAD_SUMPOOL, 4>(p, c.stream);
    }
    float* wd = c.gradws + c.net->tuw_scratch_off;
    tu_subpix_dgrad_weights_kernel<<<(16 * cv.cout * cv.cin + 255) / 256, 256, 0, c.stream>>>(c.params + cv.w, cv.cout, cv.cin, wd);
    ENDO_LAUNCH_CHECK();
    ConvParams p{};
    fill_grid(c, p, src_level);
    fill_in(c, p, c.gbuf(level), level, 0, 4 * cv.cout);
    p.sub_c = cv.cout;
    p.wgt = wd; p.w_cout = cv.cin; p.w_cin = 4 * cv.cout;
    fill_out(c, p, c.gbuf(src_level), src_level, src_c0, cv.cin);
    if (form == TuDgrad::Subpix32x8) return launch_conv_dma_vec<3, 8, 3, IN_SUBPIX, EPI_FWD, 2, 4, 2, 1, 1>(p, c.stream);
    if (form == TuDgrad::Subpix16x8) return launch_conv_dma_vec<3, 8, 3, IN_SUBPIX, EPI_FWD, 1, 2, 2, 1, 1>(p, c.stream);
    return launch_conv_dma_vec<3, 8, 3, IN_SUBPIX, EPI_FWD, 1, 1, 2, 1, 1>(p, c.stream);
}

static int64_t align_up(int64_t v, int64_t a) { return (v + a - 1) / a * a; }

}

extern "C" int endo_net_create_grouped(endo_net** out, int n, int h, int w, int groups) {
    if (!out || n <= 0 || h <= 0 || w <= 0 || groups <= 0) return ENDO_E_BADARG;
    if (groups > kMaxGroups) return ENDO_E_UNSUPPORTED;
    if ((h % 32) != 0 || (w % 32) != 0) return ENDO_E_UNSUPPORTED;
    const Table& tb = table();
    endo_net* net = new (std::nothrow) endo_net();
    if (!net) return ENDO_E_BADARG;
    net->n = n; net->h = h; net->w = w; net->groups = groups;
    net->wstream = nullptr; net->ev_fork = nullptr; net->ev_join = nullptr;
    default_options(net->opt);
    int64_t off = 0, sums = 0, pq = 0;
    for (int l = 0; l <= kLevels; ++l) {
        auto& lv = net->lv[l];
        lv.h = h >> l; lv.w = w >> l; lv.t = level_channels(l);
        lv.plane = static_cast<int64_t>(lv.h) * lv.w;
        lv.act = off; lv.grad = off;
        off += align_up(static_cast<int64_t>(n) * lv.t * lv.plane, 64);
        lv.sums = sums; sums += 2 * lv.t;
        lv.pq = pq; pq += lv.t;
    }
    const int64_t acts = off;
    net->pre_off = off; off += align_up(static_cast<int64_t>(n) * h * w, 64);
    net->saved_off = off; off += align_up(2 * tb.bn_width_total, 64);
    int64_t byte_off = off * 4;
    for (int l = 0; l < kLevels; ++l) {
        net->idx_off[l] = byte_off;
        byte_off += align_up(static_cast<int64_t>(n) * (down_in(l) + kNew) * net->lv[l + 1].plane, 256);
    }
    net->sums_off = byte_off;
    net->sums_bytes = sums * 8;
    byte_off += align_up(net->sums_bytes, 256);
    net->partial_off = byte_off / 4;
    byte_off += static_cast<int64_t>(kGrowth) * 163840 * 4;
    net->wino_off = byte_off / 4;
    byte_off += align_up(tb.wino_floats * 4, 256);
    net->wino4_off = byte_off / 4;
    byte_off += align_up(tb.wino4_floats * 4, 256);
    net->tape_floats = byte_off / 4;
    net->pq_off = acts;
    net->pq_floats = 2 * pq;
    net->scratch_off = align_up((acts + net->pq_floats) * 4, 256);
    net->slot_stride = align_up(tb.bn_width_total * 2, 32);
    net->scratch_bytes = net->slot_stride * 8 * kBnSlots;
    net->wg_scratch_off = (net->scratch_off + align_up(net->scratch_bytes, 256)) / 4;
    net->tuw_scratch_off = net->wg_scratch_off + std::max(std::max(kNsScratchFloats, kSpScratchFloats), 4 * kF34ScratchFloats);
    net->wd_off = align_up(net->tuw_scratch_off + 4 * kNew * (4 * kNew + 16), 64);
    net->gplane_off = align_up(net->wd_off + tb.wino_dgrad_floats, 64);
    net->bias_parts_off = net->gplane_off + align_up(static_cast<int64_t>(n) * h * w, 64);
    net->bias_parts_floats = static_cast<int64_t>(kBiasPartChannels) * n * groups * 32;
    {
        int launches = 1, channels = tb.first.cout;
        for (int l = 0; l < kLevels; ++l) {
            for (int j = 0; j < kLayers; ++j) { launches += 2; channels += tb.down_conv[l][j].cout + tb.up_conv[l][j].cout; }
            launches += 2; channels += tb.td_conv[l].cout + tb.tu_conv[l].cout;
        }
        for (int j = 0; j < kLayers; ++j) { ++launches; channels += tb.bott_conv[j].cout; }
        if (launches > kBiasPartLaunches || channels > kBiasPartChannels) { delete net; return ENDO_E_UNSUPPORTED; }
    }
    net->fw_parts_off = net->bias_parts_off + align_up(net->bias_parts_floats, 64);
    net->gradws_floats = net->fw_parts_off + 2 * static_cast<int64_t>(kFwPartBlocks) * 192;
    net->gs = align_up(net->tape_floats > net->gradws_floats ? net->tape_floats : net->gradws_floats, 64);
    *out = net;
    return 0;
}

extern "C" int endo_net_create(endo_net** out, int n, int h, int w) { return endo_net_create_grouped(out, n, h, w, 1); }

extern "C" int endo_net_set_option(endo_net* net, int option_id, int value) {
    if (!net || option_id < 0 || option_id >= ENDO_OPT_COUNT) return ENDO_E_BADARG;
    const int old = net->opt[option_id];
    net->opt[option_id] = value;
    return old;
}

extern "C" int endo_net_get_option(const endo_net* net, int option_id) {
    if (!net || option_id < 0 || option_id >= ENDO_OPT_COUNT) return ENDO_E_BADARG;
    return net->opt[option_id];
}

extern "C" void endo_net_destroy(endo_net* net) {
    if (!net) return;
    if (net->ev_fork) (void)hipEventDestroy(net->ev_fork);
    if (net->ev_join) (void)hipEventDestroy(net->ev_join);
    if (net->wstream) (void)hipStreamDestroy(net->wstream);
    delete net;
}
extern "C" int64_t endo_net_param_floats(void) { return table().param_floats; }
extern "C" int64_t endo_net_bn_floats(void) { return table().bn_floats; }
extern "C" int64_t endo_net_tape_floats(const endo_net* net) { return !net ? 0 : (net->groups > 1 ? net->groups * net->gs : net->tape_floats); }
extern "C" int64_t endo_net_gradws_floats(const endo_net* net) { return !net ? 0 : (net->groups > 1 ? net->groups * net->gs : net->gradws_floats); }
extern "C" int endo_net_groups(const endo_net* net) { return net ? net->groups : 0; }
extern "C" int64_t endo_net_group_stride(const endo_net* net) { return net ? net->gs : 0; }
extern "C" int64_t endo_net_param_offset(int index) {
    const Table& tb = table();
    if (index < 0 || index >= static_cast<int>(tb.param_offsets.size())) return -1;
    return tb.param_offsets[index];
}
extern "C" int64_t endo_net_bn_offset(int bn_index, int which) {
    const Table& tb = table();
    if (bn_index < 0 || bn_index >= static_cast<int>(tb.bn_order.size()) || which < 0 || which > 1) return -1;
    return tb.bn_order[bn_index]->run + which * tb.bn_order[bn_index]->c;
}
extern "C" int endo_net_level_channels(int level) { return (level < 0 || level > kLevels) ? -1 : level_channels(level); }
extern "C" int64_t endo_net_act_offset(const endo_net* net, int level) { return (!net || level < 0 || level > kLevels) ? -1 : net->lv[level].act; }

extern "C" int64_t endo_net_tape_offset(const endo_net* net, int what, int index) {
    if (!net) return -1;
    const Table& tb = table();
    switch (what) {
        case ENDO_TAPE_PRE: return net->pre_off;
        case ENDO_TAPE_BN_SAVED:
            if (index < 0 || index >= static_cast<int>(tb.bn_order.size())) return -1;
            return net->saved_off + 2 * tb.bn_order[index]->saved;
        case ENDO_TAPE_POOL:
            if (index < 0 || index >= kLevels) return -1;
            return net->idx_off[index];
        default: return -1;
    }
}

extern "C" int endo_net_fwd(endo_net* net, const float* params, float* bn_running, const float* x, float* out, float* tape,
                            int training, void* stream_) {
    if (!net || !params || !bn_running || !x || !out || !tape) return ENDO_E_BADARG;
    const Table& tb = table();
    Ctx c{net, params, bn_running, tape, nullptr, nullptr, training, static_cast<hipStream_t>(stream_)};
    const FwdPlan plan = plan_fwd(c);
    c.fwd = &plan;
    for (int g = 0; g < net->groups; ++g)
        ENDO_CHECK(hipMemsetAsync(reinterpret_cast<char*>(tape + g * net->gs) + net->sums_off, 0, net->sums_bytes, c.stream));
    if (!plan.bf16) {
        ProfScope prof(kProfSmall, c.stream, 0.0, 4.0 * (tb.wino_floats + tb.wino_floats * 9 / 16));
        WinoWeightTable wt = tb.wino;
        for (int l = 0; l < wt.layers; ++l) wt.mode[l] = plan.dense[l].chunk_weights ? 1 : 0;
        wino_fwd_weights_kernel<<<(wt.start[wt.layers] + 255) / 256, 256, 0, c.stream>>>(wt, params, tape + net->wino_off);
        ENDO_LAUNCH_CHECK();
        if (plan.wino4_weights) wino4_fwd_weights_kernel<<<(tb.wino4.start[tb.wino4.layers] + 255) / 256, 256, 0, c.stream>>>(tb.wino4, params, tape + net->wino4_off);
        ENDO_LAUNCH_CHECK();
    }
    int rc;
    {
        ConvParams p{};
        fill_grid(c, p, 0);
        p.in = x; p.in_ns = 3 * net->lv[0].plane; p.in_cs = static_cast<int>(net->lv[0].plane); p.in_w = net->w; p.cin = 3;
        p.in_gs = net->n * p.in_ns;
        p.wgt = params + tb.first.w; p.bias = params + tb.first.b; p.w_cout = kFirst; p.w_cin = 3;
        fill_out(c, p, c.act(0), 0, 48, kFirst);
        p.out_sums = c.out_sums(0, 48);
        ProfScope prof(kProfConvFirst, c.stream, conv_flops(net, 0, 3, kFirst, 3), 4.0 * c.nt() * net->lv[0].plane * (3 + kFirst));
        rc = launch_conv_dma_auto<3, 4, 3, IN_PLAIN, EPI_FWD>(p, c.stream);
        if (rc) return rc;
    }
    for (int b = 0; b < kBlocks; ++b) {
        if (b > kLevels) {
            const int i = b - kLevels - 1, l = kLevels - 1 - i;
            rc = tu_fwd(c, l, l + 1, (i == 0) ? 288 : 96 + down_in(l + 1), tb.tu_conv[i]);
            if (rc) return rc;
        }
        for (int j = 0; j < kLayers; ++j) {
            rc = dense_fwd(c, b, j);
            if (rc) return rc;
        }
        if (b < kLevels) {
            rc = td_fwd(c, b);
            if (rc) return rc;
        }
    }
    {
        const auto& lv = net->lv[0];
        const int c_first = plan.fuse_final ? 96 + down_in(0) + kGrowth * (kLayers - 1) : 0;
        ProfScope prof(kProfConvFinal, c.stream, 2.0 * c.nt() * lv.plane * 192, 4.0 * c.nt() * lv.plane * (194 - c_first));
        int bx = static_cast<int>((lv.plane / 4 + 255) / 256);
        bx = bx < 1 ? 1 : bx;
        final_fwd_kernel<<<dim3(bx, c.nt()), 256, 0, c.stream>>>(c.act(0), lv.t * lv.plane, static_cast<int>(lv.plane), 192,
                                                                 params + tb.final_.w, params + tb.final_.b, tape + net->pre_off, out,
                                                                 net->n, net->gs, c_first);
        ENDO_LAUNCH_CHECK();
    }
    return 0;
}

extern "C" int endo_net_bwd(endo_net* net, const float* params, const float* x, const float* tape, const float* grad_out,
                            float* grads, float* gradws, int training, void* stream_) {
    if (!net || !params || !x || !tape || !grad_out || !grads || !gradws) return ENDO_E_BADARG;
    const Table& tb = table();
    Ctx c{net, params, nullptr, const_cast<float*>(tape), grads, gradws, training, static_cast<hipStream_t>(stream_)};
    c.x = x;
    const BwdPlan plan = plan_bwd(c);
    c.bwd = &plan;
    BiasParts bias_parts{};
    c.bias_parts = &bias_parts;
    if (!net->wstream) {
        ENDO_CHECK(hipStreamCreateWithFlags(&net->wstream, hipStreamNonBlocking));
        ENDO_CHECK(hipEventCreateWithFlags(&net->ev_fork, hipEventDisableTiming));
        ENDO_CHECK(hipEventCreateWithFlags(&net->ev_join, hipEventDisableTiming));
    }
    for (int g = 0; g < net->groups; ++g)
        ENDO_CHECK(hipMemsetAsync(gradws + g * net->gs + net->pq_off, 0,
                                  static_cast<size_t>(net->scratch_off + net->scratch_bytes - net->pq_off * 4), c.stream));
    if (plan.dgrad_weights) {
        ProfScope prof(kProfSmall, c.stream, 0.0, 4.0 * 2.0 * tb.wino_dgrad_floats);
        int layout1_blocks = 0;
        for (int b = 0; b < kBlocks; ++b) layout1_blocks |= plan.block[b].wino3_layout ? 1 << b : 0;
        dgrad_wino_weights_kernel<<<(tb.wino_dgrad.start[tb.wino_dgrad.layers] + 255) / 256, 256, 0, c.stream>>>(tb.wino_dgrad, params, gradws + net->wd_off, layout1_blocks);
        ENDO_LAUNCH_CHECK();
    }
    int rc;
    const FinalVirt virt{gradws + net->gplane_off, params + tb.final_.w, grads + tb.final_.w};
    {
        const auto& lv = net->lv[0];
        const int materialise = plan.materialise;
        {
            Ctx cw;
            rc = c.fork_wgrad(cw, 0);
            if (rc) return rc;
            const int c_first = plan.c_first;
            int by = static_cast<int>((lv.plane + 256 * 16 - 1) / (256 * 16));
            by = by < 1 ? 1 : (by > 16 ? 16 : by);
            ProfScope prof(kProfConvFinal, cw.stream, 2.0 * c.nt() * lv.plane * (192 - c_first), 4.0 * c.nt() * lv.plane * (192 - c_first + 2));
            final_bwd_weight_kernel<<<dim3(192 - c_first + 1, by, c.nt()), 256, 0, cw.stream>>>(grad_out, tape + net->pre_off, c.act(0), lv.t * lv.plane,
                                                                         static_cast<int>(lv.plane), 192, net->n, net->gs, grads + tb.final_.w,
                                                                         grads + tb.final_.b, c_first);
            ENDO_LAUNCH_CHECK();
        }
        ProfScope prof(kProfConvFinal, c.stream, 2.0 * c.nt() * lv.plane * 192, 4.0 * c.nt() * lv.plane * (materialise + 2));
        if (plan.use_virt) {
            int bx = static_cast<int>((lv.plane + 1023) / 1024);
            final_g_kernel<<<dim3(bx, c.nt()), 256, 0, c.stream>>>(grad_out, tape + net->pre_off, gradws + net->gplane_off, static_cast<int>(lv.plane), net->n, net->gs);
            ENDO_LAUNCH_CHECK();
        }
        if (materialise > 0) {
            int bx = static_cast<int>((lv.plane + 255) / 256);
            final_bwd_data_kernel<<<dim3(bx, c.nt()), 256, 0, c.stream>>>(grad_out, tape + net->pre_off, params + tb.final_.w, c.gbuf(0),
                                                                          lv.t * lv.plane, static_cast<int>(lv.plane), materialise, net->n, net->gs, 0);
            ENDO_LAUNCH_CHECK();
        }
    }
    for (int b = kBlocks - 1; b >= 0; --b) {
        if (b < kLevels) {
            rc = td_bwd(c, b);
            if (rc) return rc;
        }
        rc = dense_block_bwd(c, b, (b == kBlocks - 1 && plan.use_virt) ? &virt : nullptr);
        if (rc) return rc;
        if (b > kLevels) {
            const int i = b - kLevels - 1, l = kLevels - 1 - i;
            rc = tu_bwd(c, l, l + 1, (i == 0) ? 288 : 96 + down_in(l + 1), tb.tu_conv[i]);
            if (rc) return rc;
        }
    }
    {
        WgradParams p = first_wgrad_params(c);
        const auto& lv = net->lv[0];
        if (plan.first == FirstWgrad::F34Prep) {
            p.prep_x = c.act(0) + 48 * lv.plane;
            p.prep_p = c.pq_p(0) + 48; p.prep_q = c.pq_q(0) + 48;
            p.prep_bias = grads + tb.first.b;
        } else {
            rc = prep_dy(c, 0, 48, kFirst, grads + tb.first.b);
            if (rc) return rc;
        }
        Ctx cw;
        rc = c.fork_wgrad(cw, 0);
        if (rc) return rc;
        ProfScope prof(kProfWgradOther, cw.stream, conv_flops(net, 0, 3, kFirst, 3), 4.0 * c.nt() * lv.plane * (3 + kFirst));
        switch (plan.first) {
            case FirstWgrad::F34Prep: rc = launch_wgrad_f34<0, true, true>(p, gradws + net->wg_scratch_off, cw.stream); break;
            case FirstWgrad::F34: rc = launch_wgrad_f34<0, true>(p, gradws + net->wg_scratch_off, cw.stream); break;
            case FirstWgrad::Taps: rc = launch_wgrad_taps<12, IN_PLAIN>(p, cw.stream); break;
            case FirstWgrad::Direct: rc = launch_wgrad<3, 3, IN_PLAIN, DY_PLAIN>(p, cw.stream); break;
        }
        if (rc) return rc;
    }
    if (bias_parts.table.n > 0) {
        ProfScope prof(kProfSmall, c.stream, 0.0, 4.0 * bias_parts.used);
        bias_reduce_kernel<<<dim3(bias_parts.table.n, 8), 256, 0, c.stream>>>(bias_parts.table);
        ENDO_LAUNCH_CHECK();
    }
    if (net->wstream) {
        ENDO_CHECK(hipEventRecord(net->ev_join, net->wstream));
        ENDO_CHECK(hipStreamWaitEvent(c.stream, net->ev_join, 0));
    }
    return 0;
}
```

### endoscopydepthestimation-pytorch_amd/models.py

```python

import ctypes

import torch
from torch import nn

from . import _lib

GROWTH = 12
LAYERS = 4
FIRST = 48
LEVELS = 5


class ConvParams(nn.Module):

    def __init__(self, cin, cout, k):
        super().__init__()
        self.weight = nn.Parameter(torch.empty(cout, cin, k, k))
        self.bias = nn.Parameter(torch.zeros(cout))
        nn.init.kaiming_uniform_(self.weight, a=5 ** 0.5)


class FusedBatchNorm2d(nn.Module):

    def __init__(self, channels):
        super().__init__()
        self.num_features = channels
        self.weight = nn.Parameter(torch.ones(channels))
        self.bias = nn.Parameter(torch.zeros(channels))
        self.register_buffer("running_mean", torch.zeros(channels))
        self.register_buffer("running_var", torch.ones(channels))
        self.register_buffer("num_batches_tracked", torch.tensor(0, dtype=torch.long))


class DenseLayer(nn.Module):
    def __init__(self, cin):
        super().__init__()
        self.norm = FusedBatchNorm2d(cin)
        self.conv = ConvParams(cin, GROWTH, 3)


class DenseBlock(nn.Module):
    def __init__(self, cin):
        super().__init__()
        self.layers = nn.ModuleList([DenseLayer(cin + j * GROWTH) for j in range(LAYERS)])


class TransitionDown(nn.Module):
    def __init__(self, channels):
        super().__init__()
        self.norm = FusedBatchNorm2d(channels)
        self.conv = ConvParams(channels, channels, 1)


class _Nearest2x(nn.Module):
    """Placeholder for nn.Upsample at index 0 of ``convTrans`` (keeps the key 'convTrans.1.*')."""


class TransitionUp(nn.Module):
    def __init__(self, channels):
        super().__init__()
        self.convTrans = nn.ModuleList([_Nearest2x(), ConvParams(channels, channels, 3)])


class Bottleneck(nn.Module):
    def __init__(self, cin):
        super().__init__()
        self.bottleneck = DenseBlock(cin)


class _NetFunction(torch.autograd.Function):

    @staticmethod
    def forward(ctx, x, anchor, net, groups=1):
        x = _lib.dev_f32(x, "FCDenseNet57 input")
        out, tape = net._run_forward(x, groups)
        ctx.net = net
        ctx.training = net.training
        ctx.tape = tape
        ctx.groups = groups
        ctx.save_for_backward(x)
        return out

    @staticmethod
    def backward(ctx, grad_out):
        if ctx.needs_input_grad[0]:
            raise RuntimeError("FCDenseNet57 on the MI355X path does not produce a gradient for its input image "
                               "(the training path never needs one, reference train.py:272-277); detach the input")
        if ctx.tape is None:
            raise RuntimeError("FCDenseNet57: the forward tape of this call was released by its first backward pass; "
                               "run the forward again (retain_graph=True is not supported for the network node)")
        (x,) = ctx.saved_tensors
        ctx.net._run_backward(x, ctx.tape, grad_out, ctx.training, ctx.groups)
        ctx.tape = None
        return None, None, None, None


class _Net16Function(torch.autograd.Function):

    @staticmethod
    def forward(ctx, x, anchor, net, half=False):
        x = _lib.dev_f32(x, "FCDenseNet57 input")
        out, tape = net._run_forward16(x, 1, half)
        ctx.half = half
        ctx.net = net
        ctx.training = net.training
        ctx.tape = tape
        ctx.shape = tuple(x.shape)
        return out

    @staticmethod
    def backward(ctx, grad_out):
        if ctx.needs_input_grad[0]:
            raise RuntimeError("FCDenseNet57 on the MI355X path does not produce a gradient for its input image; detach the input")
        if ctx.tape is None:
            raise RuntimeError("FCDenseNet57: the forward tape of this call was released by its first backward pass")
        ctx.net._run_backward16(ctx.shape, ctx.tape, grad_out, ctx.training, 1, ctx.half)
        ctx.tape = None
        return None, None, None, None


class FCDenseNet(nn.Module):

    def __init__(self, n_classes=1):
        super().__init__()
        if n_classes != 1:
            raise ValueError("the MI355X path implements the depth network (n_classes=1) only")
        self.firstconv = ConvParams(3, FIRST, 3)
        c = FIRST
        skips = []
        self.denseBlocksDown = nn.ModuleList()
        self.transDownBlocks = nn.ModuleList()
        for _ in range(LEVELS):
            self.denseBlocksDown.append(DenseBlock(c))
            c += GROWTH * LAYERS
            skips.insert(0, c)
            self.transDownBlocks.append(TransitionDown(c))
        self.bottleneck = Bottleneck(c)
        new = GROWTH * LAYERS
        self.transUpBlocks = nn.ModuleList()
        self.denseBlocksUp = nn.ModuleList()
        for i in range(LEVELS):
            self.transUpBlocks.append(TransitionUp(new))
            self.denseBlocksUp.append(DenseBlock(new + skips[i]))
        self.finalConv = ConvParams(new + skips[-1] + new, 1, 1)

        self._flat = None
        self._flat_grad = None
        self._flat_grad_full = None
        self._flat_bn = None
        self._nbt = None
        self._handles = {}
        self._gradws = {}
        self._anchor = None
        self._flatten()

    def _bn_modules(self):
        return [m for m in self.modules() if isinstance(m, FusedBatchNorm2d)]

    def _flatten(self):
        params = list(self.parameters())
        device = params[0].device
        total = sum(p.numel() for p in params)
        flat = torch.empty(total, dtype=torch.float32, device=device)
        off = 0
        offsets = []
        for p in params:
            n = p.numel()
            flat[off:off + n].copy_(p.data.reshape(-1).float())
            p.data = flat[off:off + n].view(p.shape)
            p.grad = None
            offsets.append(off)
            off += n
        self._flat, self._offsets, self._params = flat, offsets, params
        self._flat_grad = None
        self._flat_grad_full = None
        bns = self._bn_modules()
        width = sum(2 * m.num_features for m in bns)
        flat_bn = torch.empty(width, dtype=torch.float32, device=device)
        nbt = torch.empty(len(bns), dtype=torch.long, device=device)
        off = 0
        for i, m in enumerate(bns):
            c = m.num_features
            flat_bn[off:off + c].copy_(m.running_mean)
            flat_bn[off + c:off + 2 * c].copy_(m.running_var)
            nbt[i] = m.num_batches_tracked
            m._buffers["running_mean"] = flat_bn[off:off + c]
            m._buffers["running_var"] = flat_bn[off + c:off + 2 * c]
            m._buffers["num_batches_tracked"] = nbt[i]
            off += 2 * c
        self._flat_bn, self._nbt, self._bns = flat_bn, nbt, bns
        self._anchor = torch.zeros(1, device=device, requires_grad=True)
        self._gradws = {}

    def _apply(self, fn, recurse=True):
        super()._apply(fn, recurse)
        self._flatten()
        return self

    def _views_intact(self):
        base = self._flat.data_ptr()
        for p, off in zip(self._params, self._offsets):
            if p.data_ptr() != base + 4 * off:
                return False
        off = 0
        base = self._flat_bn.data_ptr()
        for m in self._bns:
            if m.running_mean.data_ptr() != base + 4 * off:
                return False
            off += 2 * m.num_features
        return True

    def flat_parameters(self):
        return self._flat

    def flat_gradients(self, create=True):
        self._attach_grads(create)
        return self._flat_grad

    def flat_gradient_bucket(self):
        self._attach_grads(True)
        return self._flat_grad_full

    def _attach_grads(self, create=True):
        if self._flat_grad is None or self._flat_grad.device != self._flat.device:
            if not create:
                return
            self._flat_grad_full = torch.zeros(self._flat.numel() + 1, dtype=torch.float32, device=self._flat.device)
            self._flat_grad = self._flat_grad_full[:self._flat.numel()]
            for p, off in zip(self._params, self._offsets):
                p.grad = self._flat_grad[off:off + p.numel()].view(p.shape)
            return
        base = self._flat_grad.data_ptr()
        intact = True
        for p, off in zip(self._params, self._offsets):
            g = p.grad
            if g is None or g.data_ptr() != base + 4 * off:
                intact = False
                break
        if not intact:
            self._flat_grad.zero_()
            for p, off in zip(self._params, self._offsets):
                p.grad = self._flat_grad[off:off + p.numel()].view(p.shape)

    def _handle(self, n, h, w, groups=1):
        key = (n, h, w, groups)
        if key not in self._handles:
            lib = _lib.load()
            if lib.endo_net_param_floats() != self._flat.numel():
                raise RuntimeError("parameter packing mismatch between Python and libendo_hip.so")
            hnd = ctypes.c_void_p()
            _lib.check(lib.endo_net_create_grouped(ctypes.byref(hnd), n, h, w, groups), "endo_net_create_grouped(%d,%d,%d,%d)" % key)
            for option_id, value in getattr(self, "_kernel_options", {}).items():
                lib.endo_net_set_option(hnd, option_id, value)
            self._handles[key] = (hnd, int(lib.endo_net_tape_floats(hnd)), int(lib.endo_net_gradws_floats(hnd)))
        return self._handles[key]

    _OPTION_DEFAULTS = {0: 5, 1: 3, 2: 2, 3: 1024, 4: 0, 5: 1, 6: 0, 7: 1, 8: 1, 9: 3}

    def set_kernel_option(self, option_id, value):
        option_id, value = int(option_id), int(value)
        if option_id not in self._OPTION_DEFAULTS:
            raise ValueError("unknown kernel option %d" % option_id)
        options = self.__dict__.setdefault("_kernel_options", {})
        old = options.get(option_id, self._OPTION_DEFAULTS[option_id])
        options[option_id] = value
        lib = _lib.load()
        for key, (hnd, _, _) in self._handles.items():
            if key[0] in ("bf16", "fp16"):
                continue
            rc = lib.endo_net_set_option(hnd, option_id, value)
            if rc < 0:
                raise RuntimeError("endo_net_set_option(%d, %d) failed: %d" % (option_id, value, rc))
        return old

    def kernel_option(self, option_id):
        return self.__dict__.get("_kernel_options", {}).get(int(option_id), self._OPTION_DEFAULTS[int(option_id)])

    def __del__(self):
        try:
            lib = _lib.load()
            for key, (hnd, _, _) in self._handles.items():
                {"bf16": lib.endo_net16_destroy, "fp16": lib.endo_net16h_destroy}.get(key[0], lib.endo_net_destroy)(hnd)
            self._handles = {}
        except Exception:
            pass

    def __getstate__(self):
        state = dict(self.__dict__)
        for key in ("_handles", "_gradws"):
            state[key] = {}
        for key in ("_flat_grad", "_flat_grad_full", "_anchor"):
            state[key] = None
        return state

    def __setstate__(self, state):
        self.__dict__.update(state)
        self._handles, self._gradws = {}, {}
        self._flatten()

    def __deepcopy__(self, memo):
        import copy
        clone = self.__class__.__new__(self.__class__)
        memo[id(self)] = clone
        state = self.__getstate__()
        for key in ("_flat", "_flat_bn", "_nbt", "_params", "_bns", "_offsets"):
            state.pop(key, None)
        clone.__dict__.update(copy.deepcopy(state, memo))
        clone._handles, clone._gradws = {}, {}
        for p in clone.parameters():
            p.grad = None
        clone._flatten()
        return clone

    def _run_forward(self, x, groups=1):
        lib = _lib.load()
        x = _lib.dev_f32(x, "FCDenseNet57 input")
        if x.dim() != 4 or x.shape[1] != 3:
            raise RuntimeError("expected N x 3 x H x W input")
        if x.device != self._flat.device:
            raise RuntimeError("model and input are on different devices; call model.cuda() first")
        if not self._views_intact():
            self._flatten()
        n, _, h, w = x.shape
        if n % groups:
            raise RuntimeError("batch of %d samples does not split into %d groups" % (n, groups))
        hnd, tape_floats, _ = self._handle(n // groups, h, w, groups)
        tape = torch.empty(tape_floats, dtype=torch.float32, device=x.device)
        out = torch.empty((n, 1, h, w), dtype=torch.float32, device=x.device)
        _lib.check(lib.endo_net_fwd(hnd, _lib.ptr(self._flat), _lib.ptr(self._flat_bn), _lib.ptr(x), _lib.ptr(out),
                                    _lib.ptr(tape), 1 if self.training else 0, _lib.stream()), "endo_net_fwd")
        if self.training:
            self._nbt.add_(groups)
        return out, tape

    def _run_backward(self, x, tape, grad_out, training, groups=1):
        lib = _lib.load()
        n, _, h, w = x.shape
        hnd, _, gradws_floats = self._handle(n // groups, h, w, groups)
        key = (n, h, w, groups)
        if key not in self._gradws:
            self._gradws[key] = torch.empty(gradws_floats, dtype=torch.float32, device=x.device)
        self._attach_grads()
        grad_out = _lib.dev_f32(grad_out, "grad_output")
        _lib.check(lib.endo_net_bwd(hnd, _lib.ptr(self._flat), _lib.ptr(x), _lib.ptr(tape), _lib.ptr(grad_out),
                                    _lib.ptr(self._flat_grad), _lib.ptr(self._gradws[key]),
                                    1 if training else 0, _lib.stream()), "endo_net_bwd")

    def forward(self, x):
        if torch.is_grad_enabled():
            return _NetFunction.apply(x, self._anchor, self)
        out, _ = self._run_forward(x)
        return out

    def forward_bf16_storage(self, x):
        if torch.is_grad_enabled():
            return _Net16Function.apply(x, self._anchor, self)
        out, _ = self._run_forward16(_lib.dev_f32(x, "FCDenseNet57 input"))
        return out

    def forward_fp16_storage(self, x):
        if torch.is_grad_enabled():
            return _Net16Function.apply(x, self._anchor, self, True)
        out, _ = self._run_forward16(_lib.dev_f32(x, "FCDenseNet57 input"), 1, True)
        return out

    @staticmethod
    def _api16(half):
        lib = _lib.load()
        prefix = "endo_net16h_" if half else "endo_net16_"
        return lambda name: getattr(lib, prefix + name)

    def set_wgrad_overlap16(self, on):
        self.__dict__["_wgrad_overlap16"] = int(on)
        for key, (hnd, _, _) in self._handles.items():
            if key[0] in ("bf16", "fp16"):
                self._api16(key[0] == "fp16")("set_wgrad_overlap")(hnd, int(on))

    def _handle16(self, n, h, w, groups=1, half=False):
        api = self._api16(half)
        key = ("fp16" if half else "bf16", n, h, w, groups)
        if key not in self._handles:
            hnd = ctypes.c_void_p()
            _lib.check(api("create")(ctypes.byref(hnd), n, h, w, groups), "endo_net16_create(%d,%d,%d,%d)" % (n, h, w, groups))
            api("set_wgrad_overlap")(hnd, int(self.__dict__.get("_wgrad_overlap16", 1)))
            self._handles[key] = (hnd, int(api("tape_bytes")(hnd)), int(api("bwd_workspace_bytes")(hnd)))
        return self._handles[key]

    def forward_pair_bf16_storage(self, x1, x2):
        x = torch.cat([_lib.dev_f32(x1, "FCDenseNet57 input"), _lib.dev_f32(x2, "FCDenseNet57 input")], dim=0)
        out, _ = self._run_forward16(x, 2)
        n = x1.shape[0]
        return out[:n], out[n:]

    def _run_forward16(self, x, groups=1, half=False):
        api = self._api16(half)
        if x.dim() != 4 or x.shape[1] != 3:
            raise RuntimeError("expected N x 3 x H x W input")
        if x.device != self._flat.device:
            raise RuntimeError("model and input are on different devices; call model.cuda() first")
        if not self._views_intact():
            self._flatten()
        n, _, h, w = x.shape
        hnd, tape_bytes, _ = self._handle16(n // groups, h, w, groups, half)
        tape = torch.empty(tape_bytes, dtype=torch.uint8, device=x.device)
        out = torch.empty((n, 1, h, w), dtype=torch.float32, device=x.device)
        with torch.no_grad():
            _lib.check(api("fwd")(hnd, _lib.ptr(self._flat), _lib.ptr(self._flat_bn), _lib.ptr(x), _lib.ptr(out), _lib.ptr(tape),
                                  1 if self.training else 0, _lib.stream()), "endo_net16_fwd")
        if self.training:
            self._nbt.add_(groups)
        return out, tape

    def _run_backward16(self, shape, tape, grad_out, training, groups=1, half=False):
        api = self._api16(half)
        n, _, h, w = shape
        hnd, _, ws_bytes = self._handle16(n // groups, h, w, groups, half)
        key = ("fp16" if half else "bf16", n // groups, h, w, groups)
        if key not in self._gradws:
            self._gradws[key] = torch.empty(ws_bytes, dtype=torch.uint8, device=tape.device)
        self._attach_grads()
        grad_out = _lib.dev_f32(grad_out, "grad_output")
        _lib.check(api("bwd")(hnd, _lib.ptr(self._flat), _lib.ptr(tape), _lib.ptr(grad_out), _lib.ptr(self._flat_grad),
                              _lib.ptr(self._gradws[key]), 1 if training else 0, _lib.stream()), "endo_net16_bwd")

    def forward_pair(self, x1, x2):
        if x1.shape != x2.shape:
            raise RuntimeError("forward_pair needs two batches of the same shape")
        x = torch.cat([_lib.dev_f32(x1, "FCDenseNet57 input"), _lib.dev_f32(x2, "FCDenseNet57 input")], dim=0)
        if torch.is_grad_enabled():
            out = _NetFunction.apply(x, self._anchor, self, 2)
        else:
            out, _ = self._run_forward(x, 2)
        n = x1.shape[0]
        return out[:n], out[n:]

    def forward_pair_packed(self, x1, x2):
        if x1.shape != x2.shape:
            raise RuntimeError("forward_pair needs two batches of the same shape")
        x = torch.cat([_lib.dev_f32(x1, "FCDenseNet57 input"), _lib.dev_f32(x2, "FCDenseNet57 input")], dim=0)
        if torch.is_grad_enabled():
            return _NetFunction.apply(x, self._anchor, self, 2)
        return self._run_forward(x, 2)[0]

    def level_buffers(self, x):
        lib = _lib.load()
        out, tape = self._run_forward(x)
        n, _, h, w = x.shape
        hnd, _, _ = self._handle(n, h, w)
        levels = []
        for lvl in range(LEVELS + 1):
            ch = lib.endo_net_level_channels(lvl)
            off = lib.endo_net_act_offset(hnd, lvl)
            hh, ww = h >> lvl, w >> lvl
            levels.append(tape[off:off + n * ch * hh * ww].view(n, ch, hh, ww))
        return out, levels


def FCDenseNet57(n_classes):
    return FCDenseNet(n_classes=n_classes)


class _DepthScaleFn(torch.autograd.Function):
    @staticmethod
    def forward(ctx, pred, sparse_depth, sparse_mask, eps):
        lib = _lib.load()
        pred = _lib.dev_f32(pred, "depth estimations")
        sd = _lib.dev_f32(sparse_depth, "sparse depths")
        sm = _lib.dev_f32(sparse_mask, "sparse masks")
        n, hw = pred.shape[0], pred.shape[1] * pred.shape[2] * pred.shape[3]
        scaled = torch.empty_like(pred)
        ratio = torch.empty((), dtype=torch.float32, device=pred.device)
        stats = torch.empty((n, 8), dtype=torch.float64, device=pred.device)
        _lib.check(lib.endo_depth_scale_fwd(_lib.ptr(pred), _lib.ptr(sd), _lib.ptr(sm), _lib.ptr(scaled), _lib.ptr(ratio),
                                            _lib.ptr(stats), n, hw, eps, _lib.stream()), "endo_depth_scale_fwd")
        ctx.save_for_backward(pred, sd, stats)
        ctx.eps = eps
        ctx.set_materialize_grads(False)
        return scaled, ratio

    @staticmethod
    def backward(ctx, grad_scaled, grad_ratio):
        lib = _lib.load()
        pred, sd, stats = ctx.saved_tensors
        if grad_scaled is None and grad_ratio is None:
            return None, None, None, None
        n, hw = pred.shape[0], pred.shape[1] * pred.shape[2] * pred.shape[3]
        gs = None if grad_scaled is None else _lib.dev_f32(grad_scaled, "grad")
        gr = None if grad_ratio is None else _lib.dev_f32(grad_ratio, "grad")
        grad_pred = torch.empty_like(pred)
        work = torch.empty((n,), dtype=torch.float64, device=pred.device)
        _lib.check(lib.endo_depth_scale_bwd(_lib.ptr(gs), _lib.ptr(gr), _lib.ptr(pred), _lib.ptr(sd), _lib.ptr(stats),
                                            _lib.ptr(grad_pred), _lib.ptr(work), n, hw, ctx.eps, _lib.stream()),
                   "endo_depth_scale_bwd")
        return grad_pred, None, None, None


class DepthScalingLayer(nn.Module):

    def __init__(self, epsilon=1.0e-8):
        super().__init__()
        self.epsilon = float(epsilon)

    def forward(self, x):
        absolute_depth_estimations, input_sparse_depths, input_weighted_sparse_masks = x
        return _DepthScaleFn.apply(absolute_depth_estimations, input_sparse_depths, input_weighted_sparse_masks,
                                   self.epsilon)


def _pose(t, r, k, n):
    t = _lib.dev_f32(t, "translation vectors").reshape(n, 3)
    r = _lib.dev_f32(r, "rotation matrices").reshape(n, 9)
    k = _lib.dev_f32(k, "intrinsic matrices").reshape(n, 9)
    return t, r, k


class _FlowFn(torch.autograd.Function):
    @staticmethod
    def forward(ctx, depth, mask, t, r, k):
        lib = _lib.load()
        depth = _lib.dev_f32(depth, "depth maps")
        mask = _lib.dev_f32(mask, "image masks")
        n, _, h, w = depth.shape
        t, r, k = _pose(t, r, k, n)
        flow = torch.empty((n, 2, h, w), dtype=torch.float32, device=depth.device)
        _lib.check(lib.endo_flow_from_depth_fwd(_lib.ptr(depth), _lib.ptr(mask), _lib.ptr(t), _lib.ptr(r), _lib.ptr(k),
                                                _lib.ptr(flow), n, h, w, _lib.stream()), "endo_flow_from_depth_fwd")
        ctx.save_for_backward(depth, mask, t, r, k)
        return flow

    @staticmethod
    def backward(ctx, grad_flow):
        lib = _lib.load()
        depth, mask, t, r, k = ctx.saved_tensors
        n, _, h, w = depth.shape
        grad_flow = _lib.dev_f32(grad_flow, "grad")
        grad_depth = torch.empty_like(depth)
        _lib.check(lib.endo_flow_from_depth_bwd(_lib.ptr(grad_flow), _lib.ptr(depth), _lib.ptr(mask), _lib.ptr(t), _lib.ptr(r),
                                                _lib.ptr(k), _lib.ptr(grad_depth), n, h, w, _lib.stream()),
                   "endo_flow_from_depth_bwd")
        return grad_depth, None, None, None, None


class FlowfromDepthLayer(nn.Module):

    def forward(self, x):
        depth_maps_1, img_masks, translation_vectors, rotation_matrices, intrinsic_matrices = x
        return _FlowFn.apply(depth_maps_1, img_masks, translation_vectors, rotation_matrices, intrinsic_matrices)


class _WarpFn(torch.autograd.Function):
    @staticmethod
    def forward(ctx, d1, d2, mask, t, r, k, eps, tile=None):
        lib = _lib.load()
        d1 = _lib.dev_f32(d1, "depth maps 1")
        d2 = _lib.dev_f32(d2, "depth maps 2")
        mask = _lib.dev_f32(mask, "image masks")
        n, _, h, w = d1.shape
        t, r, k = _pose(t, r, k, n)
        warped = torch.empty_like(d1)
        intersect = torch.empty_like(d1)
        if tile is None:
            _lib.check(lib.endo_depth_warp_fwd(_lib.ptr(d1), _lib.ptr(d2), _lib.ptr(mask), _lib.ptr(t), _lib.ptr(r), _lib.ptr(k),
                                               _lib.ptr(warped), _lib.ptr(intersect), n, h, w, eps, _lib.stream()),
                       "endo_depth_warp_fwd")
        else:
            _lib.check(lib.endo_depth_warp_fwd_tiled(_lib.ptr(d1), _lib.ptr(d2), _lib.ptr(mask), _lib.ptr(t), _lib.ptr(r), _lib.ptr(k),
                                                     _lib.ptr(warped), _lib.ptr(intersect), n, h, w, eps, int(tile[0]), int(tile[1]),
                                                     _lib.stream()), "endo_depth_warp_fwd_tiled(%d x %d)" % (tile[0], tile[1]))
        ctx.save_for_backward(d1, d2, mask, t, r, k)
        ctx.eps = eps
        ctx.tile = tile
        ctx.mark_non_differentiable(intersect)
        return warped, intersect

    @staticmethod
    def backward(ctx, grad_warped, _grad_intersect):
        lib = _lib.load()
        d1, d2, mask, t, r, k = ctx.saved_tensors
        n, _, h, w = d1.shape
        grad_warped = _lib.dev_f32(grad_warped, "grad")
        g1 = torch.empty_like(d1)
        g2 = torch.empty_like(d2)
        if ctx.tile is None:
            _lib.check(lib.endo_depth_warp_bwd(_lib.ptr(grad_warped), _lib.ptr(d1), _lib.ptr(d2), _lib.ptr(mask), _lib.ptr(t),
                                               _lib.ptr(r), _lib.ptr(k), _lib.ptr(g1), _lib.ptr(g2), n, h, w, ctx.eps,
                                               _lib.stream()), "endo_depth_warp_bwd")
        else:
            _lib.check(lib.endo_depth_warp_bwd_tiled(_lib.ptr(grad_warped), _lib.ptr(d1), _lib.ptr(d2), _lib.ptr(mask), _lib.ptr(t),
                                                     _lib.ptr(r), _lib.ptr(k), _lib.ptr(g1), _lib.ptr(g2), n, h, w, ctx.eps,
                                                     int(ctx.tile[0]), int(ctx.tile[1]), _lib.stream()), "endo_depth_warp_bwd_tiled")
        return g1, g2, None, None, None, None, None, None


class DepthWarpingLayer(nn.Module):

    def __init__(self, epsilon=1.0e-8, tile=None):
        super().__init__()
        self.epsilon = float(epsilon)
        self.tile = None if tile is None else (int(tile[0]), int(tile[1]))

    def forward(self, x):
        depth_maps_1, depth_maps_2, img_masks, translation_vectors, rotation_matrices, intrinsic_matrices = x
        warped, intersect = _WarpFn.apply(depth_maps_1, depth_maps_2, img_masks, translation_vectors, rotation_matrices,
                                          intrinsic_matrices, self.epsilon, self.tile)
        return warped, intersect
```

### include/endo_hip.h

```cpp
#ifndef ENDO_HIP_H
#define ENDO_HIP_H

#include <stdint.h>

#ifdef __cplusplus
extern "C" {
#endif

#define ENDO_E_BADARG (-1)
#define ENDO_E_UNSUPPORTED (-2)

#define ENDO_ABI_VERSION 6
int endo_abi_version(void);
const char* endo_error_string(int code);

int endo_depth_scale_fwd(const float* pred, const float* sparse_depth, const float* sparse_mask,
                         float* scaled, float* ratio, double* stats,
                         int n, int hw, float eps, void* stream);
int endo_depth_scale_bwd(const float* grad_scaled, const float* grad_ratio,
                         const float* pred, const float* sparse_depth, const double* stats,
                         float* grad_pred, double* work,
                         int n, int hw, float eps, void* stream);

int endo_flow_from_depth_fwd(const float* depth, const float* mask, const float* t, const float* R,
                             const float* K, float* flow, int n, int h, int w, void* stream);
int endo_flow_from_depth_bwd(const float* grad_flow, const float* depth, const float* mask,
                             const float* t, const float* R, const float* K, float* grad_depth,
                             int n, int h, int w, void* stream);

int endo_depth_warp_fwd(const float* depth_1, const float* depth_2, const float* mask,
                        const float* t, const float* R, const float* K,
                        float* warped, float* intersect,
                        int n, int h, int w, float eps, void* stream);
int endo_depth_warp_bwd(const float* grad_warped, const float* depth_1, const float* depth_2,
                        const float* mask, const float* t, const float* R, const float* K,
                        float* grad_d1, float* grad_d2,
                        int n, int h, int w, float eps, void* stream);
int endo_depth_warp_fwd_tiled(const float* depth_1, const float* depth_2, const float* mask,
                              const float* t, const float* R, const float* K,
                              float* warped, float* intersect,
                              int n, int h, int w, float eps, int tile_h, int tile_w, void* stream);
int endo_depth_warp_bwd_tiled(const float* grad_warped, const float* depth_1, const float* depth_2,
                              const float* mask, const float* t, const float* R, const float* K,
                              float* grad_d1, float* grad_d2,
                              int n, int h, int w, float eps, int tile_h, int tile_w, void* stream);
int endo_warp_fallback_blocks(long long* forward, long long* backward, int reset);


int endo_sparse_l1_fwd(const float* flows, const float* flows_hat, const float* mask,
                       float* loss, double* stats, int n, int c, int hw, float eps, void* stream);
int endo_sparse_l1_bwd(const float* grad_loss, const float* flows, const float* flows_hat,
                       const float* mask, const double* stats, float* grad_flows, float* grad_hat,
                       int n, int c, int hw, float eps, void* stream);

int endo_norm_dist_fwd(const float* depth, const float* warped, const float* intersect,
                       const float* K, float* loss, double* stats,
                       int n, int h, int w, float eps, void* stream);
int endo_norm_dist_bwd(const float* grad_loss, const float* depth, const float* warped,
                       const float* intersect, const float* K, const double* stats,
                       float* grad_depth, float* grad_warped,
                       int n, int h, int w, float eps, void* stream);

int endo_scale_inv_fwd(const float* pred, const float* goal, const float* boundary,
                       float* loss, double* stats, int n, int hw, float eps, void* stream);
int endo_scale_inv_bwd(const float* grad_loss, const float* pred, const float* goal,
                       const float* boundary, const double* stats,
                       float* grad_pred, float* grad_goal, int n, int hw, float eps, void* stream);

int64_t endo_loss_head_workspace_floats(int n, int h, int w);
int endo_loss_head(const float* pred_1, const float* pred_2, const float* boundaries,
                   const float* sparse_depths_1, const float* sparse_depths_2,
                   const float* sparse_depth_masks_1, const float* sparse_depth_masks_2,
                   const float* sparse_flows_1, const float* sparse_flows_2,
                   const float* sparse_flow_masks_1, const float* sparse_flow_masks_2,
                   const float* t_1_wrt_2, const float* r_1_wrt_2, const float* t_2_wrt_1, const float* r_2_wrt_1,
                   const float* intrinsics, float sfl_weight, float dcl_weight, float eps,
                   float* losses, float* grad_pred_1, float* grad_pred_2, float* workspace,
                   int n, int h, int w, void* stream);
int endo_loss_head_planes(int n, int h, int w, int64_t* offsets);

int64_t endo_warp_consistency_workspace_floats(int n, int h, int w);
int64_t endo_warp_consistency_bytes(int n, int h, int w);
int endo_warp_consistency(const float* depth_1, const float* depth_2, const float* boundaries, const float* t_1_wrt_2,
                          const float* r_1_wrt_2, const float* t_2_wrt_1, const float* r_2_wrt_1, const float* intrinsics,
                          float dcl_weight, float eps, float* loss, float* grad_depth_1, float* grad_depth_2,
                          float* workspace, int n, int h, int w, void* stream);


int endo_mask_mul(const float* a, const float* mask, float* out, int n, int c, int hw, void* stream);

typedef struct endo_net endo_net;

int endo_net_create(endo_net** out, int n, int h, int w);
int endo_net_create_grouped(endo_net** out, int n, int h, int w, int groups);
int endo_net_groups(const endo_net* net);
#define ENDO_OPT_WINO_FWD 0
#define ENDO_OPT_WINO_DGRAD 1
#define ENDO_OPT_DGRAD_VEC 2
#define ENDO_OPT_WINO_MIN_TILES 3
#define ENDO_OPT_MFMA_BF16 4
#define ENDO_OPT_WGRAD_OVERLAP 5
#define ENDO_OPT_MFMA_X3 6
#define ENDO_OPT_WGRAD_F34 7
#define ENDO_OPT_FINAL_VIRTUAL 8
#define ENDO_OPT_TD_PERSIST 9
#define ENDO_OPT_COUNT 10
int endo_net_set_option(endo_net* net, int option_id, int value);
int endo_net_get_option(const endo_net* net, int option_id);
int64_t endo_net_group_stride(const endo_net* net);
void endo_net_destroy(endo_net* net);
int64_t endo_net_param_floats(void);
int64_t endo_net_bn_floats(void);
int64_t endo_net_tape_floats(const endo_net* net);
int64_t endo_net_gradws_floats(const endo_net* net);
int64_t endo_net_param_offset(int index);
int64_t endo_net_bn_offset(int bn_index, int which );

int endo_net_fwd(endo_net* net, const float* params, float* bn_running, const float* x, float* out,
                 float* tape, int training, void* stream);
int endo_net_bwd(endo_net* net, const float* params, const float* x, const float* tape,
                 const float* grad_out, float* grads, float* gradws, int training, void* stream);
int endo_net_level_channels(int level);
int64_t endo_net_act_offset(const endo_net* net, int level);
#define ENDO_TAPE_PRE 0
#define ENDO_TAPE_BN_SAVED 1
#define ENDO_TAPE_POOL 2
int64_t endo_net_tape_offset(const endo_net* net, int what, int index);

int endo_sgd_clip_step(float* params, float* grads, float* momentum, double* norm_out,
                       int64_t count, float lr, float mu, float max_norm, float grad_scale,
                       int first_step, const float* skip_flag, void* stream);

int endo_sparse_scatter(const double* points, int n_points, const double* projections, const double* extrinsics,
                        const float* visibility, const float* clean, const uint8_t* mask, int batch, int height, int width,
                        float depth_multiplier, int32_t* winner_scratch, float* depth_masks, float* depths, float* flow_masks,
                        float* flows, void* stream);

int endo_relative_poses(const double* pair_extrinsics, int batch, double scale,
                        float* r_1_wrt_2, float* t_1_wrt_2, float* r_2_wrt_1, float* t_2_wrt_1, void* stream);

int endo_point_cloud(const float* depth, const uint8_t* color_bgr, const float* mask, const float* intrinsics, int height,
                     int width, int downsampling, int use_threshold, float min_threshold, float max_threshold,
                     int32_t* row_offsets, float* points, int32_t* count_out, void* stream);

int endo_jpeg_info(const uint8_t* data, int64_t size, int32_t* info);
int endo_jpeg_entropy_decode(const uint8_t* data, int64_t size, int16_t* blocks, int64_t capacity_blocks, uint16_t* quant);
int64_t endo_jpeg_workspace_bytes(const uint8_t* data, int64_t size);
int endo_jpeg_decode_crop(const uint8_t* data, int64_t size, double downsampling, int start_h, int end_h, int start_w,
                          int end_w, int rgb_order, uint8_t* out_hwc, float* out_chw, void* staging, void* workspace,
                          int64_t workspace_bytes, void* stream);

int endo_point_brightness(const uint8_t* imgs, int frames, int height, int width, const double* points, int n_points,
                          const double* projections, const double* extrinsics, const float* visibility, const uint8_t* mask,
                          int d, double sigma_color, double sigma_space, int32_t* valid, double* depth, float* brightness,
                          void* stream);

int endo_hsv_full(const uint8_t* src, int64_t pixels, int blue_index, uint8_t* out_u8, float* out_f32, void* stream);

typedef struct endo_augment_frame {
    int32_t colour;
    int32_t spatial;
    int32_t ksize;
    int32_t jpeg;
    int32_t noise;
    float sigma;
    uint32_t seed[2];
    uint32_t motion[2];
    int32_t reserved[6];
    uint8_t rgb_lut[256];
    uint8_t hsv_lut[3][256];
    uint16_t quant[2][64];
} endo_augment_frame;
int endo_augment_frame_bytes(void);
int64_t endo_augment_workspace_bytes(int frames, int height, int width);
int endo_augment(const uint8_t* src, const endo_augment_frame* params, int frames, int height, int width, uint8_t* out_u8,
                 float* out_f32, void* workspace, int64_t workspace_bytes, void* stream);

int64_t endo_evaluate_workspace_bytes(int frames, int height, int width);
int endo_evaluate(const float* colors, const float* boundaries, const float* predictions, const float* intrinsics, int frames,
                  int height, int width, int is_hsv, int point_cloud_downsampling, float* depth, uint8_t* panels, float* points,
                  int64_t* frame_offsets, void* workspace, int64_t workspace_bytes, void* stream);

int64_t endo_display_workspace_bytes(int n, int h, int w);
int endo_display_panel_shape(int n, int h, int w, int* rows, int* cols);
int endo_display(const float* colors_1, const float* colors_2, const float* depths_1, const float* depths_2, const float* boundaries,
                 const float* sparse_flows_1, const float* sparse_flows_2, const float* flows_1, const float* flows_2, int n, int h, int w,
                 uint8_t* out, void* workspace, int64_t workspace_bytes, void* stream);

int endo_validation_accumulate(const float* losses, int batch_index, double* means, double* history, void* stream);

int endo_depth_metrics(const float* scaled_depths, const float* sparse_depths, const float* sparse_masks, int n, int h, int w, float eps,
                       float* out, void* stream);

int64_t endo_evaluate_validation_workspace_bytes(int n, int h, int w);
int endo_evaluate_validation_panel_shape(int n, int h, int w, int* rows, int* cols);
int endo_evaluate_validation(const float* colors_1, const float* colors_2, const float* boundaries, const float* depths_1,
                             const float* depths_2, const float* sparse_depths_1, const float* sparse_depths_2,
                             const float* sparse_masks_1, const float* sparse_masks_2, const float* warped_2_to_1,
                             const float* warped_1_to_2, const float* sparse_flows_1, const float* sparse_flows_2, const float* flows_1,
                             const float* flows_2, const float* intrinsics, int n, int h, int w, float eps, int is_hsv,
                             int point_cloud_downsampling, uint8_t* panel, float* metrics, float* points, int64_t* offsets,
                             void* workspace, int64_t workspace_bytes, void* stream);

#define ENDO_PROF_FAMILIES 16
int endo_prof_enable(int family_mask);
int endo_prof_sample(int period);
int endo_prof_seen(int family, int64_t* launches);
int endo_prof_read(int family, double* total_ms, int64_t* launches, double* total_flops, double* total_bytes);
const char* endo_prof_family_name(int family);

int endo_bf16_pack_nhwc(const float* x, void* out, int n, int c, int h, int w, int t, int blk, int oc0, void* stream);
int endo_bf16_unpack_nhwc(const void* in, float* x, int n, int c, int h, int w, int t, int blk, int ic0, void* stream);
int64_t endo_bf16_conv_weight_elems(int cout, int cin, int ks);
int endo_bf16_conv_weights(const float* w, int cout, int cin, int ks, void* out, void* stream);
int endo_bf16_conv(const void* in, int in_t, int in_blk, int ic0, int cin, const float* bn, const void* wgt, const float* bias, void* out,
                   int out_t, int out_blk, int oc0, int cout, double* out_sums, int n, int h, int w, int ks, int ups, void* stream);
typedef struct endo_net16 endo_net16;
int endo_net16_create(endo_net16** out, int n_per_group, int h, int w, int groups);
void endo_net16_destroy(endo_net16* net);
int64_t endo_net16_tape_bytes(const endo_net16* net);
int endo_net16_fwd(endo_net16* net, const float* params, float* bn_running, const float* x, float* out, void* tape, int training,
                   void* stream);
int64_t endo_net16_bwd_workspace_bytes(const endo_net16* net);
int endo_net16_set_wgrad_overlap(endo_net16* net, int on);
int endo_net16h_create(endo_net16** out, int n_per_group, int h, int w, int groups);
void endo_net16h_destroy(endo_net16* net);
int64_t endo_net16h_tape_bytes(const endo_net16* net);
int endo_net16h_fwd(endo_net16* net, const float* params, float* bn_running, const float* x, float* out, void* tape, int training,
                    void* stream);
int64_t endo_net16h_bwd_workspace_bytes(const endo_net16* net);
int endo_net16h_set_wgrad_overlap(endo_net16* net, int on);
int64_t endo_net16h_offset(const endo_net16* net, int what, int index);
int endo_net16h_bwd(endo_net16* net, const float* params, const void* tape, const float* grad_out, float* grads, void* ws, int training,
                    void* stream);
int endo_f16_pack_nhwc(const float* x, void* out, int n, int c, int h, int w, int t, int blk, int oc0, void* stream);
int endo_f16_unpack_nhwc(const void* in, float* x, int n, int c, int h, int w, int t, int blk, int ic0, void* stream);
int64_t endo_net16_offset(const endo_net16* net, int what, int index);
int endo_net16_bwd(endo_net16* net, const float* params, const void* tape, const float* grad_out, float* grads, void* ws, int training,
                   void* stream);

#ifdef __cplusplus
}
#endif
#endif
```

Baseline: 512.2.

## Fold dense-block dy preparation into the persistent newmap dgrad kernel

```diff
diff --git a/endoscopydepthestimation-pytorch_amd/csrc/dgrad_newmap_kernels.h b/endoscopydepthestimation-pytorch_amd/csrc/dgrad_newmap_kernels.h
--- a/endoscopydepthestimation-pytorch_amd/csrc/dgrad_newmap_kernels.h
+++ b/endoscopydepthestimation-pytorch_amd/csrc/dgrad_newmap_kernels.h
@@ -4,7 +4,7 @@
 
 namespace endo {
 
-template <int NL>
+template <int NL, int FOLD = 0>
 struct NewMapGeom {
     using G = DgradBlockGeom<1, 2, 3, 1, 4>;
     static constexpr int kStage = 12 * G::kCS;
@@ -12,20 +12,46 @@
     static constexpr int kWPre = (kW + kConvThreads - 1) / kConvThreads;
     static constexpr int kConsts = NL * 16 * 4;
     static constexpr size_t kBytes = sizeof(float) * (2 * kStage + NL * kW + kConsts);
-    static constexpr int kBlocksPerCu = NL == 1 ? 4 : 3;
+    static constexpr int kBlocksPerCu = (NL == 1 && FOLD != 2) ? 4 : 3;
     static_assert(kBytes * kBlocksPerCu <= 160 * 1024, "LDS of the resident blocks");
     static_assert(sizeof(double) * 4 * NL * 16 * 2 <= sizeof(float) * kStage, "the final reduction aliases stage 0");
+    static constexpr int kFoldConsts = 16 * 4 + 16 * 2;
+    static_assert((kBytes + sizeof(float) * kFoldConsts) * kBlocksPerCu <= 160 * 1024, "LDS of the resident blocks with the preparation's constants");
 };
 
-template <int NL>
-__global__ void __launch_bounds__(kConvThreads, NewMapGeom<NL>::kBlocksPerCu) dgrad_newmap_kernel(const DgradBlockParams p, int tiles_y, int blocks_per_group, int tiles_per_block) {
-    using NG = NewMapGeom<NL>;
+struct NewMapFold {
+    float* dst;
+    int64_t dst_ns;
+    const float* d;
+    int64_t d_ns;
+    int d_cs;
+    const float* x;
+    float* g;
+    const float* vw;
+    const float* pq_p;
+    const float* pq_q;
+    const double* scratch[kMaxFusedLayers];
+    const float* saved[kMaxFusedLayers];
+    const float* gamma[kMaxFusedLayers];
+    float* ggamma[kMaxFusedLayers];
+    float* gbeta[kMaxFusedLayers];
+    int nl;
+    int training;
+    double count;
+    float* parts;
+};
+
+template <int NL, int FOLD = 0>
+__global__ void __launch_bounds__(kConvThreads, (NewMapGeom<NL, FOLD>::kBlocksPerCu)) dgrad_newmap_kernel(const DgradBlockParams p, int tiles_y, int blocks_per_group, int tiles_per_block, const NewMapFold f) {
+    using NG = NewMapGeom<NL, FOLD>;
     using G = typename NG::G;
     constexpr int R = 3;
     extern __shared__ __attribute__((aligned(16))) float smem[];
     float* s_g = smem;
     float* s_w = smem + 2 * NG::kStage;
     float* s_c = s_w + NL * NG::kW;
+    float* s_f = s_c + NG::kConsts;
+    double* s_fd = reinterpret_cast<double*>(s_f + 16 * 4);
 
     const int tid = threadIdx.x;
     const int lane = tid & 63;
@@ -55,7 +81,10 @@
         t_step = 1;
     }
     const int ntiles = first < t_last ? (t_last - first + t_step - 1) / t_step : 0;
-    if (ntiles <= 0) return;
+    if (ntiles <= 0) {
+        if (FOLD == 2 && tid < 12) f.parts[tid * gridDim.x + blockIdx.x] = 0.f;
+        return;
+    }
     const int64_t grp_off = p.group_n > 0 ? grp * p.gs : 0;
 
     struct Tile { int n, tx, ty, idx; };
@@ -103,6 +132,37 @@
         *reinterpret_cast<f32x4*>(s_c + tid * 4) = c4;
     }
     const float wfe = p.vg ? (co_ok ? p.vw[li] : 0.f) : 1.f;
+    if (FOLD == 2) {
+        if (tid < 12) {
+            const int c = tid;
+            float pc = f.pq_p[grp_off + c], qc = f.pq_q[grp_off + c];
+            if (f.nl > 0) {
+                double dp = 0.0, dq = 0.0;
+#pragma unroll
+                for (int j = 0; j < kMaxFusedLayers; ++j) {
+                    if (j >= f.nl) break;
+                    const double s1 = bn_slot_sum(f.scratch[j] + grp_off / 2 + 2 * c, p.slot_stride);
+                    const double s2 = bn_slot_sum(f.scratch[j] + grp_off / 2 + 2 * c + 1, p.slot_stride);
+                    if (first == 0) {
+                        atomicAdd(f.ggamma[j] + c, static_cast<float>(s2));
+                        atomicAdd(f.gbeta[j] + c, static_cast<float>(s1));
+                    }
+                    if (f.training) {
+                        const double mean = f.saved[j][grp_off + 2 * c], rstd = f.saved[j][grp_off + 2 * c + 1];
+                        const double scale = f.gamma[j][c] * rstd;
+                        const double k = scale * rstd * s2 / f.count;
+                        dp += static_cast<double>(static_cast<float>(-k));
+                        dq += static_cast<double>(static_cast<float>(-scale * s1 / f.count + k * mean));
+                    }
+                }
+                pc += static_cast<float>(dp);
+                qc += static_cast<float>(dq);
+            }
+            *reinterpret_cast<f32x4*>(s_f + c * 4) = f32x4{pc, qc, f.d_cs == 0 ? f.vw[c] : 1.f, 0.f};
+            s_fd[c] = 0.0;
+        }
+        __syncthreads();
+    }
 
     int u_ry[2], u_rx[2];
 #pragma unroll
@@ -115,6 +175,11 @@
     const unsigned kOob = 0x80000000u;
     unsigned d_vo[2] = {kOob, kOob};
     const float* d_gn = p.g;
+    int d_n = 0;
+    const bool u_in[2] = {u_ry[0] >= 1 && u_ry[0] <= G::kTileY && u_rx[0] >= G::kLeft && u_rx[0] < G::kLeft + G::kTileX,
+                          u_ry[1] >= 1 && u_ry[1] <= G::kTileY && u_rx[1] >= G::kLeft && u_rx[1] < G::kLeft + G::kTileX};
+    f32x4 fx[3][2];
+    float bsum[3] = {0.f, 0.f, 0.f};
     auto dma_tile = [&](const Tile& t) {
         const int x0 = t.tx * G::kTileX, y0 = t.ty * G::kTileY;
 #pragma unroll
@@ -124,16 +189,63 @@
             d_vo[k] = ok ? 4u * static_cast<unsigned>(gy * p.g_w + gx) : kOob;
         }
         d_gn = p.g + grp_off + static_cast<int64_t>(t.n) * p.g_ns;
+        d_n = t.n;
+    };
+    auto issue_x = [&]() {
+        const __amdgpu_buffer_rsrc_t xr = __builtin_amdgcn_make_buffer_rsrc(const_cast<float*>(f.x + grp_off + static_cast<int64_t>(d_n) * p.g_ns), 0, 12 * p.g_cs * 4, 0x00020000);
+#pragma unroll
+        for (int i = 0; i < 3; ++i) {
+            const unsigned so = 4u * static_cast<unsigned>((wave + 4 * i) * p.g_cs);
+            fx[i][0] = __builtin_bit_cast(f32x4, __builtin_amdgcn_raw_buffer_load_b128(xr, d_vo[0], so, 0));
+            fx[i][1] = __builtin_bit_cast(f32x4, __builtin_amdgcn_raw_buffer_load_b128(xr, second_unit ? d_vo[1] : kOob, so, 0));
+        }
     };
     auto issue_chunk = [&](int l, int stage) {
         float* dst = s_g + stage * NG::kStage;
-        const __amdgpu_buffer_rsrc_t gr = __builtin_amdgcn_make_buffer_rsrc(const_cast<float*>(d_gn), 0, NL * 12 * p.g_cs * 4, 0x00020000);
+        const bool raw = FOLD == 2 && l == 0;
+        const __amdgpu_buffer_rsrc_t gr = raw ? __builtin_amdgcn_make_buffer_rsrc(const_cast<float*>(f.d + grp_off + static_cast<int64_t>(d_n) * f.d_ns), 0, (11 * f.d_cs + p.g_cs) * 4, 0x00020000)
+                                              : __builtin_amdgcn_make_buffer_rsrc(const_cast<float*>(d_gn), 0, NL * 12 * p.g_cs * 4, 0x00020000);
 #pragma unroll
         for (int i = 0; i < 3; ++i) {
             const int c = wave + 4 * i;
-            const unsigned so = 4u * static_cast<unsigned>((l * 12 + c) * p.g_cs);
+            const unsigned so = 4u * static_cast<unsigned>(raw ? c * f.d_cs : (l * 12 + c) * p.g_cs);
             __builtin_amdgcn_raw_ptr_buffer_load_lds(gr, (lptr_t)(dst + c * G::kCS), 16, d_vo[0], so, 0, 0);
             if (second_unit) __builtin_amdgcn_raw_ptr_buffer_load_lds(gr, (lptr_t)(dst + c * G::kCS + 256), 16, d_vo[1], so, 0, 0);
+        }
+    };
+
+    auto form_g = [&](int stg, int n) {
+        float* dst = s_g + stg * NG::kStage;
+        const __amdgpu_buffer_rsrc_t gw = __builtin_amdgcn_make_buffer_rsrc(f.g + grp_off + static_cast<int64_t>(n) * p.g_ns, 0, 12 * p.g_cs * 4, 0x00020000);
+#pragma unroll
+        for (int i = 0; i < 3; ++i) {
+            const int c = wave + 4 * i;
+            int fo = c * 4;
+            asm volatile("" : "+v"(fo));
+            const f32x4 k4 = *reinterpret_cast<const f32x4*>(s_f + fo);
+            const unsigned co = 4u * static_cast<unsigned>(c * p.g_cs);
+            float part = 0.f;
+#pragma unroll
+            for (int k = 0; k < 2; ++k) {
+                if (k == 0 || second_unit) {
+                    const bool ok = d_vo[k] != kOob;
+                    float* sp = dst + c * G::kCS + 4 * lane + 256 * k;
+                    const f32x4 dv = *reinterpret_cast<const f32x4*>(sp);
+                    f32x4 gv;
+#pragma unroll
+                    for (int e = 0; e < 4; ++e) {
+                        float rawv = dv[e] * k4[2];
+                        asm volatile("" : "+v"(rawv));
+                        const float v = rawv + fmaf(k4[0], fx[i][k][e], k4[1]);
+                        gv[e] = ok ? v : 0.f;
+                    }
+                    *reinterpret_cast<f32x4*>(sp) = gv;
+                    const bool in = ok && u_in[k];
+                    __builtin_amdgcn_raw_buffer_store_b128(__builtin_bit_cast(u32x4_bits, gv), gw, in ? d_vo[k] + co : kOob, 0, 0);
+                    part += in ? (gv[0] + gv[1]) + (gv[2] + gv[3]) : 0.f;
+                }
+            }
+            bsum[i] += part;
         }
     };
 
@@ -144,6 +256,7 @@
     for (int r = 0; r < R; ++r) lo_r[r] = static_cast<unsigned>(li * p.cs + (wy + r) * p.w + lane_x);
     const unsigned lo_ch = static_cast<unsigned>(li * p.cs);
     int64_t cur_off = 0, po_off = 0, cur_voff = 0;
+    int64_t cur_doff = 0, po_doff = 0;
     unsigned cur_rows = 0, po_rows = 0;
     bool cur_full = false, po_full = false;
     auto begin_tile = [&](const Tile& t) {
@@ -151,6 +264,7 @@
         cur_full = y0 + G::kTileY <= p.h && x0 + G::kTileX <= p.w;
         cur_off = grp_off + static_cast<int64_t>(t.n) * p.ns + y0 * p.w + x0;
         cur_voff = grp_off + static_cast<int64_t>(t.n) * p.cs + y0 * p.w + x0;
+        if (FOLD) cur_doff = grp_off + static_cast<int64_t>(t.n) * f.dst_ns + y0 * p.w + x0;
         const float* xb = p.x + cur_off;
         const float* ob = p.vg ? p.vg + cur_voff : p.out + cur_off;
         if (cur_full) {
@@ -179,7 +293,7 @@
     };
 
     auto store_results = [&]() {
-        float* ob = p.out + po_off;
+        float* ob = FOLD ? f.dst + po_doff : p.out + po_off;
         if (po_full) {
             if (co_ok) {
 #pragma unroll
@@ -207,7 +321,9 @@
     for (int t = 0; t < ntiles; ++t) {
 #pragma unroll
         for (int l = 0; l < NL; ++l) {
+            if (FOLD == 2 && l == 0) issue_x();
             asm volatile("s_waitcnt vmcnt(0)" ::: "memory");
+            if (FOLD == 2 && l == 0) form_g(stage, cur.n);
             __syncthreads();
             if (l == 0) {
                 if (t > 0) {
@@ -292,12 +408,21 @@
                         dc[r][e] = old + total[r][e];
                     }
                 po_off = cur_off;
+                po_doff = cur_doff;
                 po_rows = cur_rows;
                 po_full = cur_full;
                 cur = nxt;
                 advance(nxt);
                 if (++tiles_since_flush == kFlushTiles) {
                     tiles_since_flush = 0;
+                    if (FOLD == 2) {
+#pragma unroll
+                        for (int i = 0; i < 3; ++i) {
+                            const double v = wave_sum(static_cast<double>(bsum[i]));
+                            if (lane == 0) s_fd[wave + 4 * i] += v;
+                            bsum[i] = 0.f;
+                        }
+                    }
 #pragma unroll
                     for (int k = 0; k < NL; ++k) {
                         ds1[k] += static_cast<double>(fs1[k]); ds2[k] += static_cast<double>(fs2[k]);
@@ -310,6 +435,13 @@
         }
     }
     store_results();
+    if (FOLD == 2) {
+#pragma unroll
+        for (int i = 0; i < 3; ++i) {
+            const double v = wave_sum(static_cast<double>(bsum[i]));
+            if (lane == 0) f.parts[(wave + 4 * i) * gridDim.x + blockIdx.x] = static_cast<float>(s_fd[wave + 4 * i] + v);
+        }
+    }
 
     __syncthreads();
     double* red = reinterpret_cast<double*>(smem);
@@ -342,19 +474,33 @@
     return p.count <= 16 && p.acc_from == 0 && 36ll * p.g_cs * 4 < (1ll << 31) && (16ll * p.cs + static_cast<int64_t>(p.h) * p.w) * 4 < (1ll << 32);
 }
 
-template <int NL>
-inline int launch_dgrad_newmap(DgradBlockParams p, hipStream_t stream) {
-    using NG = NewMapGeom<NL>;
+struct NewMapGrid { int tiles_x, tiles_y, blocks_per_group, tiles_per_block, blocks; };
+
+template <int NL, int FOLD = 0>
+inline NewMapGrid dgrad_newmap_grid(const DgradBlockParams& p) {
+    using NG = NewMapGeom<NL, FOLD>;
     using G = typename NG::G;
-    p.tiles_x = (p.w + G::kTileX - 1) / G::kTileX;
-    const int tiles_y = (p.h + G::kTileY - 1) / G::kTileY;
+    NewMapGrid g{};
+    g.tiles_x = (p.w + G::kTileX - 1) / G::kTileX;
+    g.tiles_y = (p.h + G::kTileY - 1) / G::kTileY;
     const int groups = p.group_n > 0 ? p.n / p.group_n : 1;
-    const int tiles_per_group = p.tiles_x * tiles_y * (p.group_n > 0 ? p.group_n : p.n);
+    const int tiles_per_group = g.tiles_x * g.tiles_y * (p.group_n > 0 ? p.group_n : p.n);
     const int resident = device_cu_count() * NG::kBlocksPerCu / groups;
-    const int tiles_per_block = (tiles_per_group + resident - 1) / resident;
-    int blocks_per_group = (tiles_per_group + tiles_per_block - 1) / tiles_per_block;
-    blocks_per_group = (blocks_per_group + 7) / 8 * 8;
-    return launch_dyn(dgrad_newmap_kernel<NL>, dim3(groups * blocks_per_group), kConvThreads, NG::kBytes, stream, p, tiles_y, blocks_per_group, tiles_per_block);
+    g.tiles_per_block = (tiles_per_group + resident - 1) / resident;
+    g.blocks_per_group = (tiles_per_group + g.tiles_per_block - 1) / g.tiles_per_block;
+    g.blocks_per_group = (g.blocks_per_group + 7) / 8 * 8;
+    g.blocks = groups * g.blocks_per_group;
+    return g;
 }
-
+constexpr int kNewMapMaxBlocks = 2048;
+
+template <int NL, int FOLD = 0>
+inline int launch_dgrad_newmap(DgradBlockParams p, hipStream_t stream, const NewMapFold& f = NewMapFold{}) {
+    using NG = NewMapGeom<NL, FOLD>;
+    const NewMapGrid g = dgrad_newmap_grid<NL, FOLD>(p);
+    p.tiles_x = g.tiles_x;
+    const size_t bytes = NG::kBytes + (FOLD == 2 ? sizeof(float) * NG::kFoldConsts : 0);
+    return launch_dyn(dgrad_newmap_kernel<NL, FOLD>, dim3(g.blocks), kConvThreads, bytes, stream, p, g.tiles_y, g.blocks_per_group, g.tiles_per_block, f);
 }
+
+}
diff --git a/endoscopydepthestimation-pytorch_amd/csrc/net.hip b/endoscopydepthestimation-pytorch_amd/csrc/net.hip
--- a/endoscopydepthestimation-pytorch_amd/csrc/net.hip
+++ b/endoscopydepthestimation-pytorch_amd/csrc/net.hip
@@ -157,6 +157,8 @@
     int64_t bias_parts_off;
     int64_t fw_parts_off;
     int64_t bias_parts_floats;
+    int64_t fold_off;
+    int64_t fold_set_floats;
     int64_t gradws_floats;
     hipStream_t wstream;
     hipEvent_t ev_fork, ev_join;
@@ -168,6 +170,7 @@
 
 constexpr int kBiasPartChannels = 2048;
 constexpr int kBiasPartLaunches = 64;
+constexpr int kFoldPasses = 3 * (2 * kLevels + 1);
 constexpr int kFwPartBlocks = 512;
 struct BiasReduceTable {
     int n;
@@ -186,7 +189,7 @@
     float* gbeta[4];
 };
 
-__global__ void __launch_bounds__(256) prep_dy_kernel(float* __restrict__ dbuf, const float* __restrict__ x, int64_t ns, int plane,
+__global__ void __launch_bounds__(256) prep_dy_kernel(float* dbuf, const float* dsrc, int64_t src_ns, const float* __restrict__ x, int64_t ns, int plane,
                                                       const float* __restrict__ pq_p, const float* __restrict__ pq_q,
                                                       float* bias_grad, int group_n, int64_t gs, const BnFin4 fin, int nl,
                                                       double count, int training, int64_t slot_stride,
@@ -219,6 +222,7 @@
         qc += static_cast<float>(dq);
     }
     const int64_t base = grp * gs + n * ns + static_cast<int64_t>(c) * plane;
+    const float* dsrc_c = dsrc + (grp * gs + n * src_ns + static_cast<int64_t>(c) * plane);
     const float* vg_n = vg ? vg + grp * gs + static_cast<int64_t>(n) * plane : nullptr;
     const float wf = vg ? vw[c] : 0.f;
     float part = 0.f;
@@ -226,8 +230,8 @@
         const int stride = gridDim.x * blockDim.x * 4;
         int i = (blockIdx.x * blockDim.x + threadIdx.x) * 4;
         for (; i + stride < plane; i += 2 * stride) {
-            f32x4 g0 = *reinterpret_cast<const f32x4*>(dbuf + base + i);
-            f32x4 g1 = *reinterpret_cast<const f32x4*>(dbuf + base + i + stride);
+            f32x4 g0 = *reinterpret_cast<const f32x4*>(dsrc_c + i);
+            f32x4 g1 = *reinterpret_cast<const f32x4*>(dsrc_c + i + stride);
             const f32x4 x0 = *reinterpret_cast<const f32x4*>(x + base + i);
             const f32x4 x1 = *reinterpret_cast<const f32x4*>(x + base + i + stride);
 #pragma unroll
@@ -238,7 +242,7 @@
             *reinterpret_cast<f32x4*>(dbuf + base + i + stride) = g1;
         }
         for (; i < plane; i += stride) {
-            f32x4 g = *reinterpret_cast<const f32x4*>(dbuf + base + i);
+            f32x4 g = *reinterpret_cast<const f32x4*>(dsrc_c + i);
             const f32x4 xv = *reinterpret_cast<const f32x4*>(x + base + i);
 #pragma unroll
             for (int e = 0; e < 4; ++e) { g[e] += fmaf(pc, xv[e], qc); part += g[e]; }
@@ -251,7 +255,7 @@
                 const f32x4 gv = *reinterpret_cast<const f32x4*>(vg_n + i);
                 g = f32x4{gv[0] * wf, gv[1] * wf, gv[2] * wf, gv[3] * wf};
             } else {
-                g = *reinterpret_cast<const f32x4*>(dbuf + base + i);
+                g = *reinterpret_cast<const f32x4*>(dsrc_c + i);
             }
             const f32x4 xv = *reinterpret_cast<const f32x4*>(x + base + i);
 #pragma unroll
@@ -260,7 +264,7 @@
         }
     } else {
         for (int i = blockIdx.x * blockDim.x + threadIdx.x; i < plane; i += gridDim.x * blockDim.x) {
-            const float g = (vg_n ? vg_n[i] * wf : dbuf[base + i]) + fmaf(pc, x[base + i], qc);
+            const float g = (vg_n ? vg_n[i] * wf : dsrc_c[i]) + fmaf(pc, x[base + i], qc);
             dbuf[base + i] = g;
             part += g;
         }
@@ -535,6 +539,7 @@
         NewMap newmap[kLayers];
         BasePass base;
         bool wino3_layout;
+        bool fold;
     } block[kBlocks];
     DenseWgrad wgrad[kDense];
     bool td_wgrad_dma[kLevels];
@@ -640,6 +645,7 @@
     opt[ENDO_OPT_WGRAD_F34] = 1;
     opt[ENDO_OPT_FINAL_VIRTUAL] = 1;
     opt[ENDO_OPT_TD_PERSIST] = 3;
+    opt[ENDO_OPT_PREP_FOLD] = 1;
 }
 static int bf16_mask(const int* opt) { const int v = opt[ENDO_OPT_MFMA_BF16]; return v == 1 ? 7 : (v >> 1); }
 
@@ -818,7 +824,8 @@
 
 struct FinalVirt { const float* vg; const float* vw; float* gw; };
 
-static int prep_dy(const Ctx& c, int level, int c0, int count, float* bias_grad, const BnFin4* fin = nullptr, int nl = 0, const FinalVirt* fv = nullptr) {
+static int prep_dy(const Ctx& c, int level, int c0, int count, float* bias_grad, const BnFin4* fin = nullptr, int nl = 0, const FinalVirt* fv = nullptr,
+                   const float* src = nullptr) {
     const auto& lv = c.net->lv[level];
     BnFin4 none{};
     int bx = static_cast<int>((lv.plane + 4095) / 4096);
@@ -833,7 +840,8 @@
         bp.used += need;
     }
     ProfScope prof(kProfSmall, c.stream, 0.0, 12.0 * c.nt() * lv.plane * count);
-    prep_dy_kernel<<<dim3(bx, count, c.nt()), 256, 0, c.stream>>>(c.gbuf(level) + c0 * lv.plane, c.act(level) + c0 * lv.plane,
+    float* dbuf = c.gbuf(level) + c0 * lv.plane;
+    prep_dy_kernel<<<dim3(bx, count, c.nt()), 256, 0, c.stream>>>(dbuf, src ? src : dbuf, src ? count * lv.plane : lv.t * lv.plane, c.act(level) + c0 * lv.plane,
                                                                      lv.t * lv.plane, static_cast<int>(lv.plane), c.pq_p(level) + c0,
                                                                      c.pq_q(level) + c0, bias_grad, c.net->n, c.net->gs, fin ? *fin : none, fin ? nl : 0,
                                                                      static_cast<double>(c.net->n) * lv.h * lv.w, c.training, c.net->slot_stride,
@@ -1016,6 +1024,12 @@
             bl.newmap[j] = (pl.bf16_dgrad && vec) ? NewMap::Bf16 : (vec && opt[ENDO_OPT_DGRAD_VEC] >= 2 && dgrad_newmap_ok(p)) ? NewMap::Persistent
                          : (vec && opt[ENDO_OPT_DGRAD_VEC] != 0) ? NewMap::Vec16 : NewMap::Dword;
         }
+        {
+            const DgradBlockParams p1 = newmap_params(c, k, kLayers - 1);
+            const int grid = std::max(dgrad_newmap_grid<1>(p1).blocks, dgrad_newmap_grid<2>(p1).blocks);
+            bl.fold = opt[ENDO_OPT_PREP_FOLD] != 0 && bl.fused && tile_count(c, k.level, 32, 6) >= min_tiles && grid <= kNewMapMaxBlocks;
+            for (int j = 1; j < kLayers; ++j) bl.fold = bl.fold && bl.newmap[j] == NewMap::Persistent;
+        }
         for (int j = 0; j < kLayers; ++j) {
             const WgradParams p = dense_wgrad_params(c, k, j);
             pl.wgrad[b * kLayers + j] = (f34 && wgrad_f34_ok(p, f34_min_tiles)) ? DenseWgrad::F34 : wgrad_nsplit_ok(p) ? (x3 ? DenseWgrad::X3 : DenseWgrad::NSplit)
@@ -1097,6 +1111,11 @@
 }
 
 template <int NL>
+static int launch_newmap_fold(bool prepares, const DgradBlockParams& p, const NewMapFold& f, hipStream_t stream) {
+    return prepares ? launch_dgrad_newmap<NL, 2>(p, stream, f) : launch_dgrad_newmap<NL, 1>(p, stream, f);
+}
+
+template <int NL>
 static int launch_newmap(NewMap form, const DgradBlockParams& p, hipStream_t stream) {
     switch (form) {
         case NewMap::Bf16: return launch_dgrad_block<NL, 2, 3, 1, 0, 1, 4, 1>(p, stream);
@@ -1123,23 +1142,37 @@
     BnFin4 pending{};
     int pending_nl = 0;
     F34ReduceBatch red{};
+    float* const sets[2] = {c.gradws + c.net->fold_off, c.gradws + c.net->fold_off + c.net->fold_set_floats};
+    const int64_t set_ns = kGrowth * lv.plane;
+    int set = 0;
     for (int j = kLayers - 1; j >= 0; --j) {
-        int rc = prep_dy(c, level, new0 + kGrowth * j, kGrowth, c.grads + k.cv[j].b, &pending, pending_nl, (fv && j == kLayers - 1) ? fv : nullptr);
-        if (rc) return rc;
+        const FinalVirt* fvj = (fv && j == kLayers - 1) ? fv : nullptr;
+        const bool in_pass = bl.fold && j > 0 && (j < kLayers - 1 || fvj);
+        const float* raw = (bl.fold && j < kLayers - 1) ? sets[set ^ 1] : nullptr;
+        int rc = 0;
+        if (!in_pass) {
+            rc = prep_dy(c, level, new0 + kGrowth * j, kGrowth, c.grads + k.cv[j].b, &pending, pending_nl, fvj, raw);
+            if (rc) return rc;
+        }
         const bool defer = c.bwd->overlap == 2;
-        if (!defer || j == 0) {
+        auto fork = [&]() -> int {
+            if (defer && j != 0) return 0;
             Ctx cw;
-            rc = c.fork_wgrad(cw, level);
-            if (rc) return rc;
+            int r = c.fork_wgrad(cw, level);
+            if (r) return r;
             for (int jj = defer ? kLayers - 1 : j; jj >= j; --jj) {
-                rc = dense_wgrad(cw, b, jj, &red, jj);
-                if (rc) return rc;
+                r = dense_wgrad(cw, b, jj, &red, jj);
+                if (r) return r;
             }
             if (j == 0 && red.count > 0) {
                 ProfScope prof(kProfSmall, cw.stream, 0.0, 0.0);
-                rc = launch_wgrad_f34_reduce_batch(red, cw.stream);
-                if (rc) return rc;
+                r = launch_wgrad_f34_reduce_batch(red, cw.stream);
             }
+            return r;
+        };
+        if (!in_pass) {
+            rc = fork();
+            if (rc) return rc;
         }
         if (j > 0) {
             const int nl = kLayers - j;
@@ -1148,10 +1181,41 @@
             if (fv) { p.vg = fv->vg; p.vw = fv->vw + ic0 + p.w_ci_off; }
             ProfScope prof(kProfDgradDense, c.stream, 2.0 * c.nt() * lv.plane * kGrowth * kGrowth * 9 * nl,
                            4.0 * c.nt() * lv.plane * (3.0 * kGrowth + kGrowth * nl));
-            rc = nl == 1 ? launch_newmap<1>(bl.newmap[j], p, c.stream) : nl == 2 ? launch_newmap<2>(bl.newmap[j], p, c.stream) : launch_newmap<3>(bl.newmap[j], p, c.stream);
+            if (bl.fold) {
+                NewMapFold f{};
+                f.dst = sets[set]; f.dst_ns = set_ns;
+                if (in_pass) {
+                    const int ch = new0 + kGrowth * j;
+                    f.d = fvj ? fvj->vg : raw; f.d_ns = fvj ? lv.plane : set_ns; f.d_cs = fvj ? 0 : static_cast<int>(lv.plane);
+                    f.x = c.act(level) + ch * lv.plane;
+                    f.g = c.gbuf(level) + ch * lv.plane;
+                    f.vw = fvj ? fvj->vw + ch : nullptr;
+                    f.pq_p = c.pq_p(level) + ch; f.pq_q = c.pq_q(level) + ch;
+                    for (int l = 0; l < pending_nl; ++l) {
+                        f.scratch[l] = pending.scratch[l]; f.saved[l] = pending.saved[l]; f.gamma[l] = pending.gamma[l];
+                        f.ggamma[l] = pending.ggamma[l]; f.gbeta[l] = pending.gbeta[l];
+                    }
+                    f.nl = pending_nl; f.training = c.training; f.count = static_cast<double>(c.net->n) * lv.h * lv.w;
+                    const int blocks = nl == 1 ? dgrad_newmap_grid<1, 2>(p).blocks : nl == 2 ? dgrad_newmap_grid<2, 2>(p).blocks : dgrad_newmap_grid<3, 2>(p).blocks;
+                    BiasParts& bp = *c.bias_parts;
+                    const int64_t need = static_cast<int64_t>(kGrowth) * blocks;
+                    if (bp.table.n >= kBiasPartLaunches || bp.used + need > c.net->bias_parts_floats) return ENDO_E_UNSUPPORTED;
+                    f.parts = c.gradws + c.net->bias_parts_off + bp.used;
+                    bp.table.e[bp.table.n++] = {f.parts, c.grads + k.cv[j].b, kGrowth, blocks};
+                    bp.used += need;
+                }
+                rc = nl == 1 ? launch_newmap_fold<1>(in_pass, p, f, c.stream) : nl == 2 ? launch_newmap_fold<2>(in_pass, p, f, c.stream) : launch_newmap_fold<3>(in_pass, p, f, c.stream);
+                set ^= 1;
+            } else {
+                rc = nl == 1 ? launch_newmap<1>(bl.newmap[j], p, c.stream) : nl == 2 ? launch_newmap<2>(bl.newmap[j], p, c.stream) : launch_newmap<3>(bl.newmap[j], p, c.stream);
+            }
             if (rc) return rc;
             pending = a;
             pending_nl = nl;
+        }
+        if (in_pass) {
+            rc = fork();
+            if (rc) return rc;
         }
     }
     {
@@ -1318,7 +1382,8 @@
     net->wd_off = align_up(net->tuw_scratch_off + 4 * kNew * (4 * kNew + 16), 64);
     net->gplane_off = align_up(net->wd_off + tb.wino_dgrad_floats, 64);
     net->bias_parts_off = net->gplane_off + align_up(static_cast<int64_t>(n) * h * w, 64);
-    net->bias_parts_floats = static_cast<int64_t>(kBiasPartChannels) * n * groups * 32;
+    net->bias_parts_floats = static_cast<int64_t>(kBiasPartChannels) * n * groups * 32
+                           + static_cast<int64_t>(kFoldPasses) * kGrowth * kNewMapMaxBlocks;
     {
         int launches = 1, channels = tb.first.cout;
         for (int l = 0; l < kLevels; ++l) {
@@ -1329,7 +1394,9 @@
         if (launches > kBiasPartLaunches || channels > kBiasPartChannels) { delete net; return ENDO_E_UNSUPPORTED; }
     }
     net->fw_parts_off = net->bias_parts_off + align_up(net->bias_parts_floats, 64);
-    net->gradws_floats = net->fw_parts_off + 2 * static_cast<int64_t>(kFwPartBlocks) * 192;
+    net->fold_off = align_up(net->fw_parts_off + 2 * static_cast<int64_t>(kFwPartBlocks) * 192, 64);
+    net->fold_set_floats = align_up(static_cast<int64_t>(n) * kGrowth * net->lv[0].plane, 64);
+    net->gradws_floats = net->fold_off + 2 * net->fold_set_floats;
     net->gs = align_up(net->tape_floats > net->gradws_floats ? net->tape_floats : net->gradws_floats, 64);
     *out = net;
     return 0;
diff --git a/endoscopydepthestimation-pytorch_amd/models.py b/endoscopydepthestimation-pytorch_amd/models.py
--- a/endoscopydepthestimation-pytorch_amd/models.py
+++ b/endoscopydepthestimation-pytorch_amd/models.py
@@ -256,7 +256,7 @@
             self._handles[key] = (hnd, int(lib.endo_net_tape_floats(hnd)), int(lib.endo_net_gradws_floats(hnd)))
         return self._handles[key]
 
-    _OPTION_DEFAULTS = {0: 5, 1: 3, 2: 2, 3: 1024, 4: 0, 5: 1, 6: 0, 7: 1, 8: 1, 9: 3}
+    _OPTION_DEFAULTS = {0: 5, 1: 3, 2: 2, 3: 1024, 4: 0, 5: 1, 6: 0, 7: 1, 8: 1, 9: 3, 10: 1}
 
     def set_kernel_option(self, option_id, value):
         option_id, value = int(option_id), int(value)
diff --git a/include/endo_hip.h b/include/endo_hip.h
--- a/include/endo_hip.h
+++ b/include/endo_hip.h
@@ -104,7 +104,8 @@
 #define ENDO_OPT_WGRAD_F34 7
 #define ENDO_OPT_FINAL_VIRTUAL 8
 #define ENDO_OPT_TD_PERSIST 9
-#define ENDO_OPT_COUNT 10
+#define ENDO_OPT_PREP_FOLD 10
+#define ENDO_OPT_COUNT 11
 int endo_net_set_option(endo_net* net, int option_id, int value);
 int endo_net_get_option(const endo_net* net, int option_id);
 int64_t endo_net_group_stride(const endo_net* net);
```

Result: no change. 509.8 (-0.5%).
